# 0xPolygonZero/proof-protocol-decoder

Measured on AMD Instinct MI355X. Metric: txn-proofs/sec (whole node), 256-txn synthetic block, higher is better.
Workload: dtype u64 (Goldilocks field)

## Files before the change

include/bpg.h:

```cpp
#ifndef BPG_H
#define BPG_H
#include <stddef.h>
#include <stdint.h>

#ifdef __cplusplus
extern "C" {
#endif

typedef enum {
  BP_OK = 0,
  BP_ERR_ABORTED = -1,
  BP_ERR_INVALID_INPUT = -2,
  BP_ERR_RANGE = -3,
  BP_ERR_DEVICE = -4,
  BP_ERR_VERIFY = -5,
  BP_ERR_UNSUPPORTED = -6
} bp_status;

const char* bp_last_error(void);
const char* bp_version(void);
int bp_device_count(void);
int bp_use_blocking_sync(int device);
int bp_host_wait_mode(int device);



#define BP_NTT_MAX_COLS 65535u

enum { BP_NTT_FWD_BR2NAT = 0, BP_NTT_INV_NAT2BR = 1, BP_NTT_FWD_NAT = 2, BP_NTT_INV_NAT = 3 };
int bp_ntt_batch(uint64_t* d_cols, uint32_t log_n, uint32_t n_cols, uint64_t col_stride, int dir,
                 void* stream);

int bp_intt_batch(const uint64_t* d_values, uint64_t in_stride, uint64_t* d_coeffs_out, uint64_t out_stride,
                  uint32_t log_n, uint32_t n_cols, void* stream);

int bp_lde_batch(const uint64_t* d_in, uint64_t in_stride, uint64_t* d_coeffs_out, uint64_t coeffs_stride,
                 uint64_t* d_lde_out, uint64_t lde_stride, uint32_t log_n, uint32_t rate_bits,
                 uint32_t n_cols, int from_coeffs, void* stream);

int bp_debug_copy_u64(const uint64_t* d_in, uint64_t* d_out, uint64_t n, void* stream);

int bp_debug_field_ops(const uint64_t* d_a, const uint64_t* d_b, uint64_t* d_out, uint64_t n, void* stream);
int bp_debug_mul_pow2(const uint64_t* d_a, uint64_t* d_out, uint64_t n, void* stream);

void bp_tune_quad_threshold(uint64_t n_perms);
void bp_tune_merkle_fused(int mode);
void bp_tune_merkle_wide(int log2_parents);
void bp_tune_poseidon_mx(int on);
void bp_tune_poseidon_mx_sets(int sets);
void bp_tune_poseidon_grouped(int on);
void bp_tune_assume_loaded(int mode);
void bp_tune_rec_batch(int n);
void bp_tune_side_lanes(int n);
void bp_tune_rec_riders(int on);
void bp_tune_witness_threads(int n);
void bp_tune_host_wait(int mode);
void bp_tune_host_poseidon(int mode);
int bp_debug_poseidon_host(uint64_t* states, size_t n);
void bp_tune_k5_spread(int on);
uint32_t bp_debug_poseidon_group_ops(uint32_t K);
int bp_debug_poseidon_group_tables(uint32_t K, uint32_t r0, uint8_t* out_ops, int32_t* out_cform, int32_t* out_cmain,
                                   int32_t* out_max_plane_sum);

void bp_tune_ntt_split(int mode);
void bp_tune_ntt_mx(int mode);
void bp_tune_reset(void);
int bp_debug_tune_state(char* buf, size_t cap);
int bp_debug_ntt_mx_tables(int kind, int inverse, uint8_t* out_a, int32_t* out_c, uint64_t* out_tw256,
                           uint64_t* out_tw16);
int bp_debug_poseidon_mx_cin(uint32_t* out);

int bp_poseidon_perm_batch(uint64_t* d_states, uint64_t n, void* stream);

uint64_t bp_merkle_digest_words(uint32_t log_leaves, uint32_t cap_height);
int bp_merkle_commit(const uint64_t* d_lde, uint64_t lde_stride, uint32_t n_cols, uint32_t log_n,
                     uint32_t rate_bits, uint32_t cap_height, uint64_t* d_digests, void* stream);

struct bp_stark_cfg;
typedef struct bp_air_family {
  uint32_t first_index, count;
  uint32_t kind;
  uint32_t degree;
} bp_air_family;
typedef struct bp_air_desc {
  uint32_t air_id;
  char name[24];
  uint32_t fixed_n_cols;
  uint32_t n_const_max;
  uint32_t degree;
  uint32_t n_cols, n_aux;
  uint32_t n_air_constraints, n_ctl_constraints;
  uint32_t n_units;
  uint32_t n_families;
  bp_air_family families[24];
} bp_air_desc;
uint32_t bp_air_count(void);
int bp_air_describe(uint32_t air_id, uint32_t n_cols, uint32_t n_const, uint32_t deg_pow, bp_air_desc* out);

int bp_air_register(const uint64_t* program, size_t n_words, uint32_t* air_id_out);
int bp_air_unregister(uint32_t air_id);
int bp_air_program_digest(uint32_t air_id, uint8_t out[32]);

uint64_t bp_quotient_scratch_words(uint32_t air_id, const struct bp_stark_cfg* shape);
int bp_quotient_eval(uint32_t air_id, const struct bp_stark_cfg* shape, const uint64_t* d_trace_lde,
                     const uint64_t* d_aux_lde, const uint64_t* d_const_lde, const uint64_t ctl[4],
                     const uint64_t alphas[2], uint64_t* d_scratch, uint64_t* d_qvals_out, void* stream);

int bp_air_port_products(uint32_t air_id, const struct bp_stark_cfg* shape, const uint64_t* d_trace, uint64_t stride,
                         const uint64_t* d_consts, const uint64_t pub[4], const uint64_t ctl[4], uint64_t* d_aux_out, void* stream);

int bp_debug_air_aux(uint32_t air_id, const struct bp_stark_cfg* shape, const uint64_t* d_trace, const uint64_t ctl[4],
                     uint64_t* d_aux_out, void* stream);

typedef struct bp_air_violation {
  uint32_t row, constraint, family, kind;
  uint64_t value;
} bp_air_violation;
int bp_air_check_trace(uint32_t air_id, const struct bp_stark_cfg* shape, const uint64_t* d_trace, uint64_t stride,
                       const uint64_t* d_consts, const uint64_t pub[4], uint32_t max_rows, uint64_t* n_violated_rows,
                       uint32_t* rows_out, bp_air_violation* viol_out, uint32_t max_viol, uint32_t* n_viol, void* stream);
int bp_air_check_trace_host(uint32_t air_id, const struct bp_stark_cfg* shape, const uint64_t* trace, uint64_t stride,
                            const uint64_t* consts, const uint64_t pub[4], uint32_t max_rows, uint64_t* n_violated_rows,
                            uint32_t* rows_out, bp_air_violation* viol_out, uint32_t max_viol, uint32_t* n_viol);

int bp_keccak_trace(const uint64_t* d_inputs, uint64_t seed, uint32_t log_n, uint64_t* d_trace_out, void* stream);
int bp_logic_trace(const uint64_t* d_inputs, uint64_t seed, uint32_t log_n, uint64_t* d_trace_out, void* stream);
int bp_memory_trace(const uint64_t* d_inputs, uint64_t seed, uint32_t log_n, uint64_t* d_trace_out, void* stream);
int bp_arithmetic_trace(const uint64_t* d_inputs, uint64_t seed, uint32_t log_n, uint64_t* d_trace_out, void* stream);
int bp_byte_packing_trace(const uint64_t* d_inputs, uint64_t seed, uint32_t log_n, uint64_t* d_trace_out, void* stream);
int bp_keccak_sponge_trace(const uint64_t* d_inputs, uint64_t seed, uint32_t log_n, uint64_t* d_trace_out, void* stream);
int bp_arithmetic_mul_trace(const uint64_t* d_inputs, uint64_t seed, uint32_t log_n, uint64_t* d_trace_out, void* stream);

typedef struct bp_plonk_layout {
  uint32_t pi_len, n_paths, path_depth, path_pi0;
  uint32_t leaf_len;
} bp_plonk_layout;
int bp_plonk_constants(uint64_t seed, uint32_t log_n, const bp_plonk_layout* layout, uint64_t* d_consts_out, void* stream);
int bp_plonk_trace(const uint64_t* d_consts, uint64_t seed, const uint64_t* pi, const bp_plonk_layout* layout, const uint64_t* paths,
                   uint32_t log_n, uint64_t* d_trace_out, void* stream);

int bp_fri_fold(const uint64_t* d_values, uint32_t log_nl, uint32_t rate_bits, uint32_t arity_bits, uint64_t shift,
                const uint64_t beta[2], uint64_t* d_out, void* stream);

int bp_openings(const uint64_t* d_coeffs, uint64_t stride, uint32_t log_n, uint32_t n_cols, const uint64_t z0[2],
                const uint64_t z1[2], uint64_t* d_pw_scratch, uint64_t* d_out, void* stream);

int bp_pow_grind(const uint64_t state[12], uint32_t pos, uint32_t bits, uint64_t* nonce_out, void* stream);

typedef struct bp_stark_cfg {
  uint32_t log_n, n_cols, n_const, deg_pow, rate_bits, cap_height, num_queries, pow_bits, arity_bits,
      final_poly_bits;
} bp_stark_cfg;
int bp_stark_prove_synthetic(const bp_stark_cfg* cfg, uint64_t seed, uint64_t const_seed, int device,
                             uint8_t** out, size_t* out_len);
int bp_stark_prove_air(uint32_t air_id, const bp_stark_cfg* cfg, uint64_t seed, uint64_t const_seed, int device,
                       uint8_t** out, size_t* out_len);
int bp_stark_prove_trace(uint32_t air_id, const bp_stark_cfg* cfg, const uint64_t* d_trace, uint64_t stride,
                         const uint64_t* d_consts, const uint64_t* pub, int device, uint8_t** out, size_t* out_len);
int bp_stark_verify_air(uint32_t air_id, const bp_stark_cfg* cfg, const uint64_t* const_cap, const uint8_t* proof,
                        size_t len);
void bp_stark_public_inputs(uint64_t seed, uint64_t out[4]);
void bp_stark_public_input_list(uint64_t seed, uint64_t out[4]);
int bp_stark_verify_air_pub(uint32_t air_id, const bp_stark_cfg* cfg, const uint64_t* const_cap, const uint64_t* pub,
                            const uint8_t* proof, size_t len);
typedef struct bp_set_table {
  uint32_t air_id;
  bp_stark_cfg cfg;
  const uint64_t* d_trace;
  uint64_t stride;
  const uint64_t* d_consts;
  const uint64_t* pub;
} bp_set_table;
typedef struct bp_set_port {
  uint32_t table, port;
} bp_set_port;
typedef struct bp_set_link {
  uint32_t n_looking;
  bp_set_port looking[8];
  bp_set_port looked;
} bp_set_link;
#define BP_SET_SKIP_LINK_CHECK 1u
int bp_stark_prove_table_set(const bp_set_table* tables, uint32_t n_tables, const bp_set_link* links, uint32_t n_links,
                             uint32_t flags, int device, uint8_t** out, size_t* out_len);
int bp_stark_verify_table_set(const bp_set_table* statement, uint32_t n_tables, const uint64_t* const* const_caps,
                              const bp_set_link* links, uint32_t n_links, const uint8_t* proof, size_t len);
void bp_release_cached_memory(void);
void bp_free_buffer(uint8_t* buf);

#define BP_NUM_TABLES 7

typedef struct bp_config {
  uint32_t table_log_lo[BP_NUM_TABLES], table_log_hi[BP_NUM_TABLES];
  uint32_t stark_rate_bits, stark_cap_height, stark_num_queries, stark_pow_bits, arity_bits, final_poly_bits;
  uint32_t rec_log_n, rec_n_cols, rec_n_const, rec_rate_bits, rec_num_queries, rec_pow_bits;
  uint32_t shrink_depth;
  uint32_t rec_air_id;
  int32_t device;
  uint32_t n_workers;
  uint64_t arena_bytes;
} bp_config;
// ... 161 lines not shown
```

proof_protocol_decoder_amd/_lib.py:

```python
import ctypes as C
import os

_HERE = os.path.dirname(os.path.abspath(__file__))
_PATH = os.environ.get("BPG_LIBBPG") or os.path.join(_HERE, "lib", "libbpg.so")

BP_OK = 0
STATUS_NAMES = {0: "BP_OK", -1: "BP_ERR_ABORTED", -2: "BP_ERR_INVALID_INPUT", -3: "BP_ERR_RANGE",
                -4: "BP_ERR_DEVICE", -5: "BP_ERR_VERIFY", -6: "BP_ERR_UNSUPPORTED"}


class BpgError(RuntimeError):

    def __init__(self, code, message):
        super().__init__("%s: %s" % (STATUS_NAMES.get(code, str(code)), message))
        self.code = code
        self.message = message


class StarkCfg(C.Structure):
    _fields_ = [(n, C.c_uint32) for n in ("log_n", "n_cols", "n_const", "deg_pow", "rate_bits", "cap_height",
                                           "num_queries", "pow_bits", "arity_bits", "final_poly_bits")]


class AirFamily(C.Structure):
    _fields_ = [(n, C.c_uint32) for n in ("first_index", "count", "kind", "degree")]


class AirDesc(C.Structure):
    _fields_ = ([("air_id", C.c_uint32), ("name", C.c_char * 24)]
                + [(n, C.c_uint32) for n in ("fixed_n_cols", "n_const_max", "degree", "n_cols", "n_aux",
                                             "n_air_constraints", "n_ctl_constraints", "n_units", "n_families")]
                + [("families", AirFamily * 24)])


class SetTable(C.Structure):
    _fields_ = [("air_id", C.c_uint32), ("cfg", StarkCfg), ("d_trace", C.c_void_p), ("stride", C.c_uint64),
                ("d_consts", C.c_void_p), ("pub", C.POINTER(C.c_uint64))]


class SetPort(C.Structure):
    _fields_ = [("table", C.c_uint32), ("port", C.c_uint32)]


class SetLink(C.Structure):
    _fields_ = [("n_looking", C.c_uint32), ("looking", SetPort * 8), ("looked", SetPort)]


BP_SET_SKIP_LINK_CHECK = 1


class AirViolation(C.Structure):
    _fields_ = [(n, C.c_uint32) for n in ("row", "constraint", "family", "kind")] + [("value", C.c_uint64)]


def take_buffer(ptr, length):
    try:
        return C.string_at(ptr, length.value)
    finally:
        lib().bp_free_buffer(ptr)


def lib_path():
    return _PATH


KNOBS = ("quad_threshold", "assume_loaded", "merkle_fused", "merkle_wide", "poseidon_mx", "poseidon_mx_sets",
         "poseidon_grouped", "ntt_mx", "ntt_split", "k5_spread", "host_wait", "host_poseidon", "rec_batch",
         "witness_threads", "side_lanes")

_lib = None


def lib():
    global _lib
    if _lib is not None:
        return _lib
    if not os.path.exists(_PATH):
        raise ImportError(
            "libbpg.so not built at %s -- run `python -c 'import __graft_entry__ as g; g.build()'` "
            "(hipcc --offload-arch=gfx950). There is no CPU fallback for the hot path." % _PATH)
    L = C.CDLL(_PATH)
    vp, u32, u64, i = C.c_void_p, C.c_uint32, C.c_uint64, C.c_int
    L.bp_last_error.restype = C.c_char_p
    L.bp_version.restype = C.c_char_p
    L.bp_device_count.restype = i
    L.bp_ntt_batch.argtypes = [vp, u32, u32, u64, i, vp]
    L.bp_intt_batch.argtypes = [vp, u64, vp, u64, u32, u32, vp]
    L.bp_lde_batch.argtypes = [vp, u64, vp, u64, vp, u64, u32, u32, u32, i, vp]
    L.bp_poseidon_perm_batch.argtypes = [vp, u64, vp]
    L.bp_debug_field_ops.argtypes = [vp, vp, vp, u64, vp]
    L.bp_debug_mul_pow2.argtypes = [vp, vp, u64, vp]
    L.bp_quotient_scratch_words.argtypes = [u32, C.POINTER(StarkCfg)]
    L.bp_quotient_scratch_words.restype = u64
    L.bp_quotient_eval.argtypes = [u32, C.POINTER(StarkCfg), vp, vp, vp, C.POINTER(u64), C.POINTER(u64), vp, vp, vp]
    L.bp_air_count.restype = u32
    L.bp_air_describe.argtypes = [u32, u32, u32, u32, C.POINTER(AirDesc)]
    check_args = [u32, C.POINTER(StarkCfg), vp, u64, vp, C.POINTER(u64), u32, C.POINTER(u64), C.POINTER(u32),
                  C.POINTER(AirViolation), u32, C.POINTER(u32)]
    L.bp_air_check_trace.argtypes = check_args + [vp]
    L.bp_air_check_trace_host.argtypes = check_args
    L.bp_keccak_trace.argtypes = [vp, u64, u32, vp, vp]
    L.bp_logic_trace.argtypes = [vp, u64, u32, vp, vp]
    L.bp_memory_trace.argtypes = [vp, u64, u32, vp, vp]
    L.bp_arithmetic_trace.argtypes = [vp, u64, u32, vp, vp]
    L.bp_byte_packing_trace.argtypes = [vp, u64, u32, vp, vp]
    L.bp_keccak_sponge_trace.argtypes = [vp, u64, u32, vp, vp]
    L.bp_arithmetic_mul_trace.argtypes = [vp, u64, u32, vp, vp]
    L.bp_stark_verify_air.argtypes = [u32, C.POINTER(StarkCfg), C.POINTER(u64), C.c_char_p, C.c_size_t]
    L.bp_stark_prove_air.argtypes = [u32, C.POINTER(StarkCfg), u64, u64, i, C.POINTER(C.POINTER(C.c_uint8)),
                                     C.POINTER(C.c_size_t)]
    L.bp_stark_verify_air_pub.argtypes = [u32, C.POINTER(StarkCfg), C.POINTER(u64), C.POINTER(u64), C.c_char_p, C.c_size_t]
    L.bp_stark_prove_trace.argtypes = [u32, C.POINTER(StarkCfg), vp, u64, vp, C.POINTER(u64), i, C.POINTER(C.POINTER(C.c_uint8)),
                                       C.POINTER(C.c_size_t)]
    L.bp_debug_air_aux.argtypes = [u32, C.POINTER(StarkCfg), vp, C.POINTER(u64), vp, vp]
    L.bp_air_port_products.argtypes = [u32, C.POINTER(StarkCfg), vp, u64, vp, C.POINTER(u64), C.POINTER(u64), vp, vp]
    L.bp_stark_prove_table_set.argtypes = [C.POINTER(SetTable), u32, C.POINTER(SetLink), u32, u32, i,
                                           C.POINTER(C.POINTER(C.c_uint8)), C.POINTER(C.c_size_t)]
    L.bp_stark_verify_table_set.argtypes = [C.POINTER(SetTable), u32, C.POINTER(C.POINTER(u64)), C.POINTER(SetLink), u32,
                                            C.c_char_p, C.c_size_t]
    L.bp_air_register.argtypes = [vp, C.c_size_t, C.POINTER(u32)]
    L.bp_air_unregister.argtypes = [u32]
    L.bp_air_program_digest.argtypes = [u32, C.c_char_p]
    L.bp_fri_fold.argtypes = [vp, u32, u32, u32, u64, C.POINTER(u64), vp, vp]
    L.bp_openings.argtypes = [vp, u64, u32, u32, C.POINTER(u64), C.POINTER(u64), vp, vp, vp]
    L.bp_pow_grind.argtypes = [C.POINTER(u64), u32, u32, C.POINTER(u64), vp]
    L.bp_merkle_digest_words.argtypes = [u32, u32]
    L.bp_merkle_digest_words.restype = u64
    L.bp_merkle_commit.argtypes = [vp, u64, u32, u32, u32, u32, vp, vp]
    L.bp_stark_prove_synthetic.argtypes = [C.POINTER(StarkCfg), u64, u64, i, C.POINTER(C.POINTER(C.c_uint8)),
                                           C.POINTER(C.c_size_t)]
    L.bp_free_buffer.argtypes = [C.POINTER(C.c_uint8)]
    L.bp_free_buffer.restype = None
    for knob in KNOBS:
        fn = getattr(L, "bp_tune_" + knob)
        fn.argtypes = [u64 if knob == "quad_threshold" else i]
        fn.restype = None
    L.bp_tune_reset.argtypes = []
    L.bp_tune_reset.restype = None
    L.bp_debug_tune_state.argtypes = [C.c_char_p, C.c_size_t]
    _lib = L
    return L


def check(rc):
    if rc != BP_OK:
        raise BpgError(rc, lib().bp_last_error().decode("utf-8", "replace"))
```

proof_protocol_decoder_amd/csrc/hash_kernels.hip:

```cpp
#include <atomic>
#include <cstring>
#include <memory>
#include <mutex>
#include <vector>
#include "common.hpp"
#include "poseidon.cuh"
#include "poseidon_mx.cuh"
#include "stark_kernels.hpp"
#include "tune.hpp"

namespace {

__global__ void __launch_bounds__(256) perm_batch_kernel(uint64_t* __restrict__ states, uint64_t n) {
  uint64_t i = blockIdx.x * (uint64_t)blockDim.x + threadIdx.x;
  if (i >= n) return;
  uint64_t s[12];
#pragma unroll
  for (int k = 0; k < 12; k++) s[k] = states[i * 12 + k];
  poseidon::permute(s);
#pragma unroll
  for (int k = 0; k < 12; k++) states[i * 12 + k] = gl::canon(s[k]);
}

__global__ void __launch_bounds__(256) __attribute__((amdgpu_waves_per_eu(4, 8)))
// ... 258 lines not shown
      const uint64_t leaf = ((uint64_t)gl::bitrev(t, rate_bits) << log_n) | gl::bitrev(mm, log_n);
      digests[leaf * 4 + kb] = gl::canon(e[m][0]);
    }
  }
}

template <int NS, bool GR>
__global__ void BPG_MX_BOUNDS
merkle_level_mx_kernel(const uint64_t* __restrict__ child, uint64_t* __restrict__ parent, uint64_t n_parents,
                       uint64_t* __restrict__ mirror, uint64_t dig_bstride, const uint32_t* __restrict__ gtab) {
  if (gridDim.x * gridDim.z <= 64) __builtin_amdgcn_s_setprio(3);
  child += blockIdx.z * dig_bstride;
  parent += blockIdx.z * dig_bstride;
  if (mirror) mirror += blockIdx.z * n_parents * 4;
  BPG_MX_TABLES(NS, GR, gtab)
  const poseidon::mx::Ctx c = poseidon::mx::make_ctx(cin);
  const uint64_t base = ((uint64_t)blockIdx.x * 4 + (threadIdx.x >> 6)) * (16 * NS) + (threadIdx.x & 15);
  uint64_t e[NS][3];
#pragma unroll
  for (int m = 0; m < NS; m++) {
    const uint64_t i = base + 16 * m < n_parents ? base + 16 * m : n_parents - 1;
    e[m][0] = child[i * 8 + c.kb];
    e[m][1] = child[i * 8 + 4 + c.kb];
    e[m][2] = 0;
  }
  BPG_MX_PERMUTE(NS, GR, e, c, gtab)
#pragma unroll
  for (int m = 0; m < NS; m++) {
    const uint64_t i = base + 16 * m;
    if (i < n_parents) {
      const uint64_t d = gl::canon(e[m][0]);
      parent[i * 4 + c.kb] = d;
      if (mirror) mirror[i * 4 + c.kb] = d;
    }
  }
}

__global__ void __launch_bounds__(256)
merkle_subtree_mx_kernel(const uint64_t* __restrict__ child, uint64_t* __restrict__ out, uint64_t n_parents,
                         uint32_t levels, uint64_t* __restrict__ mirror, uint64_t dig_bstride) {
  if (gridDim.x * gridDim.z <= 64) __builtin_amdgcn_s_setprio(3);
  child += blockIdx.z * dig_bstride;
  out += blockIdx.z * dig_bstride;
  if (mirror) mirror += blockIdx.z * ((n_parents >> (levels - 1)) * 4);
  __shared__ __attribute__((aligned(16))) uint32_t cin[poseidon::mx::CIN_WORDS];
  __shared__ uint64_t sm[2][64 * 4];
  poseidon::mx::build_cin(cin);
  __syncthreads();
  const poseidon::mx::Ctx c = poseidon::mx::make_ctx(cin);
  const uint32_t wave = threadIdx.x >> 6, n = threadIdx.x & 15;
  uint64_t level_parents = n_parents;
  uint32_t wg_parents = n_parents < 64 ? (uint32_t)n_parents : 64u;
  uint64_t wg_first = (uint64_t)blockIdx.x * 64;
  uint64_t* dst = out;
  for (uint32_t l = 0; l < levels; l++) {
    if (wave * 16 < wg_parents) {
      const uint32_t q = wave * 16 + n, qc = q < wg_parents ? q : wg_parents - 1;
      uint64_t e[1][3];
      if (l == 0) {
        e[0][0] = child[(wg_first + qc) * 8 + c.kb];
        e[0][1] = child[(wg_first + qc) * 8 + 4 + c.kb];
      } else {
        e[0][0] = sm[(l - 1) & 1][(2 * qc) * 4 + c.kb];
        e[0][1] = sm[(l - 1) & 1][(2 * qc + 1) * 4 + c.kb];
      }
      e[0][2] = 0;
      poseidon::mx::permute<1>(e, c);
      if (q < wg_parents) {
        const uint64_t d = gl::canon(e[0][0]);
        dst[(wg_first + q) * 4 + c.kb] = d;
        if (mirror && l + 1 == levels) mirror[(wg_first + q) * 4 + c.kb] = d;
        sm[l & 1][q * 4 + c.kb] = d;
      }
    }
    __syncthreads();
    dst += level_parents * 4;
    level_parents >>= 1;
    wg_parents >>= 1;
    wg_first >>= 1;
  }
}

__global__ void __launch_bounds__(256)
merkle_subtree_wide_kernel(const uint64_t* __restrict__ child, uint64_t* __restrict__ out, uint64_t n_parents,
                           uint32_t levels, uint64_t* __restrict__ mirror, uint64_t dig_bstride) {
  if (gridDim.x * gridDim.z <= 64) __builtin_amdgcn_s_setprio(3);
  child += blockIdx.z * dig_bstride;
  out += blockIdx.z * dig_bstride;
  if (mirror) mirror += blockIdx.z * ((n_parents >> (levels - 1)) * 4);
  __shared__ __attribute__((aligned(16))) uint32_t cin[poseidon::mx::CIN_WORDS];
  __shared__ uint64_t sm[2][256 * 4];
  poseidon::mx::build_cin(cin);
  __syncthreads();
  const poseidon::mx::Ctx c = poseidon::mx::make_ctx(cin);
  const uint32_t wave = threadIdx.x >> 6, n = threadIdx.x & 15;
  uint64_t level_parents = n_parents;
  uint32_t wg_parents = n_parents < 256 ? (uint32_t)n_parents : 256u;
  uint64_t wg_first = (uint64_t)blockIdx.x * 256;
  uint64_t* dst = out;
  for (uint32_t l = 0; l < levels; l++) {
    const uint64_t* prev = sm[(l - 1) & 1];
    if (wg_parents >= 64) {
      if (wave * 64 < wg_parents) {
        uint64_t e[4][3];
#pragma unroll
        for (int m = 0; m < 4; m++) {
          const uint32_t q = wave * 64 + 16 * m + n;
          if (l == 0) {
            e[m][0] = child[(wg_first + q) * 8 + c.kb];
            e[m][1] = child[(wg_first + q) * 8 + 4 + c.kb];
          } else {
            e[m][0] = prev[(2 * q) * 4 + c.kb];
            e[m][1] = prev[(2 * q + 1) * 4 + c.kb];
          }
          e[m][2] = 0;
        }
        poseidon::mx::permute<4>(e, c);
#pragma unroll
        for (int m = 0; m < 4; m++) {
          const uint32_t q = wave * 64 + 16 * m + n;
          const uint64_t d = gl::canon(e[m][0]);
          dst[(wg_first + q) * 4 + c.kb] = d;
          if (mirror && l + 1 == levels) mirror[(wg_first + q) * 4 + c.kb] = d;
          sm[l & 1][q * 4 + c.kb] = d;
        }
      }
    } else if (wave * 16 < wg_parents) {
      const uint32_t q = wave * 16 + n, qc = q < wg_parents ? q : wg_parents - 1;
      uint64_t e[1][3];
      if (l == 0) {
        e[0][0] = child[(wg_first + qc) * 8 + c.kb];
        e[0][1] = child[(wg_first + qc) * 8 + 4 + c.kb];
      } else {
        e[0][0] = prev[(2 * qc) * 4 + c.kb];
        e[0][1] = prev[(2 * qc + 1) * 4 + c.kb];
      }
      e[0][2] = 0;
      poseidon::mx::permute<1>(e, c);
      if (q < wg_parents) {
        const uint64_t d = gl::canon(e[0][0]);
        dst[(wg_first + q) * 4 + c.kb] = d;
        if (mirror && l + 1 == levels) mirror[(wg_first + q) * 4 + c.kb] = d;
        sm[l & 1][q * 4 + c.kb] = d;
      }
    }
    __syncthreads();
    dst += level_parents * 4;
    level_parents >>= 1;
    wg_parents >>= 1;
    wg_first >>= 1;
  }
}

template <int K>
__device__ __forceinline__ void mul_pow2_planes(const uint64_t (&x)[4], uint64_t* __restrict__ out, uint64_t n, uint64_t i0) {
  uint64_t r4[4], r3[3];
  const uint64_t x3[3] = {x[1], x[2], x[3]};
  gl::mul_pow2_n<12 * K, 4>(x, r4);
  __builtin_amdgcn_sched_barrier(0);
  gl::mul_pow2_n<12 * K, 3>(x3, r3);
  __builtin_amdgcn_sched_barrier(0);
#pragma unroll
  for (int k = 0; k < 4; k++) {
    const uint64_t i = i0 + k;
    if (i >= n) break;
    out[(3 * (K - 1) + 0) * n + i] = gl::canon(r4[k]);
    out[(3 * (K - 1) + 1) * n + i] = k ? gl::canon(r3[k - 1]) : gl::canon(r4[0]);
    out[(3 * (K - 1) + 2) * n + i] = gl::canon(gl::mul_pow2(x[k], 12 * K));
  }
  if constexpr (K < 7) mul_pow2_planes<K + 1>(x, out, n, i0);
}
__global__ void __launch_bounds__(256) mul_pow2_kernel(const uint64_t* __restrict__ a, uint64_t* __restrict__ out, uint64_t n) {
  const uint64_t i0 = (blockIdx.x * (uint64_t)blockDim.x + threadIdx.x) * 4;
  if (i0 >= n) return;
  uint64_t x[4];
#pragma unroll
  for (int k = 0; k < 4; k++) x[k] = a[i0 + k < n ? i0 + k : n - 1];
  mul_pow2_planes<1>(x, out, n, i0);
}

__global__ void __launch_bounds__(256)
calib_copy_u64_kernel(const uint64_t* __restrict__ in, uint64_t* __restrict__ out, uint64_t n) {
  uint64_t i = blockIdx.x * (uint64_t)blockDim.x + threadIdx.x;
  const uint64_t stride = (uint64_t)gridDim.x * blockDim.x;
  for (; i < n; i += stride) out[i] = in[i];
}

__global__ void __launch_bounds__(256) field_ops_kernel(const uint64_t* __restrict__ a, const uint64_t* __restrict__ b,
                                                        uint64_t* __restrict__ out, uint64_t n) {
  const uint64_t i0 = (blockIdx.x * (uint64_t)blockDim.x + threadIdx.x) * 4;
  if (i0 >= n) return;
  uint64_t x[4], y[4];
#pragma unroll
  for (int k = 0; k < 4; k++) {
    const uint64_t i = i0 + k < n ? i0 + k : n - 1;
    x[k] = a[i];
    y[k] = b[i];
  }
  uint64_t r4[4], r3[3];
  gl::mul_n<4>(x, y, r4);
  __builtin_amdgcn_sched_barrier(0);
  const uint64_t x3[3] = {x[1], x[2], x[3]}, y3[3] = {y[1], y[2], y[3]};
  gl::mul_n<3>(x3, y3, r3);
  __builtin_amdgcn_sched_barrier(0);
  gl::DotAcc d[4] = {gl::dot_zero(), gl::dot_zero(), gl::dot_zero(), gl::dot_zero()};
  gl::dot_mad4(d, x, y);
  __builtin_amdgcn_sched_barrier(0);
  gl::dot_mad4(d, y, x);
  __builtin_amdgcn_sched_barrier(0);
  const uint64_t yy[4] = {y[0], y[0], y[0], y[0]};
  gl::dot_mad4(d, x, yy);
  __builtin_amdgcn_sched_barrier(0);
  uint64_t cy[4] = {y[0], y[1], y[2], y[3]}, sum4[4], dif4[4], cx4[4] = {x[0], x[1], x[2], x[3]};
  gl::canon_n<4>(cy);
  __builtin_amdgcn_sched_barrier(0);
  gl::add_n<4>(x, cy, sum4);
  __builtin_amdgcn_sched_barrier(0);
  gl::sub_n<4>(x, cy, dif4);
  __builtin_amdgcn_sched_barrier(0);
  gl::canon_n<4>(cx4);
  __builtin_amdgcn_sched_barrier(0);
#pragma unroll
  for (int k = 0; k < 4; k++) {
    const uint64_t i = i0 + k;
    if (i >= n) break;
    const uint64_t cb = gl::canon(y[k]);
    out[0 * n + i] = gl::canon(gl::mul(x[k], y[k]));
    out[1 * n + i] = gl::canon(r4[k]);
    out[2 * n + i] = k ? gl::canon(r3[k - 1]) : gl::canon(r4[0]);
    uint64_t lo, hi;
    gl::mul_wide(x[k], y[k], lo, hi);
    out[3 * n + i] = gl::canon(gl::reduce128(lo, hi));
    out[4 * n + i] = gl::canon(gl::add(x[k], cb));
    out[5 * n + i] = gl::canon(gl::sub(x[k], cb));
    out[6 * n + i] = gl::dot_reduce(d[k]);
    out[7 * n + i] = gl::canon(gl::mul7(x[k]));
    out[8 * n + i] = gl::inv(gl::canon(x[k]));
    const gl::Ext e = gl::mul(gl::Ext{gl::canon(x[k]), cb}, gl::Ext{cb, gl::canon(x[k] ^ y[k])});
    out[9 * n + i] = e.c0;
    out[10 * n + i] = e.c1;
    out[11 * n + i] = gl::canon(sum4[k]);
    out[12 * n + i] = gl::canon(dif4[k]);
    out[13 * n + i] = cx4[k];
    out[14 * n + i] = cy[k];
  }
}

}

namespace bpg {

static std::atomic<int> g_active_provers{0};
void prover_active(int delta) { g_active_provers.fetch_add(delta, std::memory_order_relaxed); }
int provers_active() { return g_active_provers.load(std::memory_order_relaxed); }
bool device_loaded() {
  const int a = tune().assume_loaded.load(std::memory_order_relaxed);
  return a < 0 ? g_active_provers.load(std::memory_order_relaxed) >= 6 : a != 0;
}
bool poseidon_mx() { return tune().poseidon_mx.load(std::memory_order_relaxed) != 0; }
uint64_t quad_threshold() {
  const uint64_t t = tune().quad_threshold.load(std::memory_order_relaxed);
  if (t) return t;
  const bool loaded = device_loaded();
  if (poseidon_mx()) return (uint64_t)1 << (loaded ? 13 : 19);
  return (uint64_t)1 << (loaded ? 13 : 17);
}
int mx_sets(uint64_t n) {
  if (!poseidon_mx()) return 0;
  const int f = tune().poseidon_mx_sets.load(std::memory_order_relaxed);
  if (f) return f;
  const uint64_t t = quad_threshold();
  return n >= t ? 4 : (n >= t / 2 ? 2 : 1);
}
static std::mutex g_group_mu;
static const uint32_t* g_group_dev[16] = {};
static std::atomic<int> g_group_state[16];
static std::vector<uint32_t>* g_group_image = nullptr;

static bool build_group_image() {
  namespace pg = poseidon::group;
  namespace gx = poseidon::mx::grp;
  if (g_group_image) return true;
  auto img = std::make_unique<std::vector<uint32_t>>(gx::IMAGE_WORDS, 0);
  for (int g = 0; g < gx::N_GROUPS; g++) {
    pg::Tables t;
    uint32_t* c = img->data() + gx::OPS_WORDS + g * gx::C_WORDS;
    if (g < 2) {
      if (!pg::build(gx::K, 4 + gx::K * g, &t) || (int)t.ops.size() != gx::LAY.n_ops * 1024) return false;
      if (g == 0) std::memcpy(img->data(), t.ops.data(), t.ops.size());
      else if (std::memcmp(img->data(), t.ops.data(), t.ops.size()) != 0) return false;
    } else {
      constexpr pg::Layout L6 = pg::layout(gx::SHORT_K);
      if (!pg::build(gx::SHORT_K, 20, &t) || (int)t.ops.size() != L6.n_ops * 1024) return false;
      const uint8_t* o8 = reinterpret_cast<const uint8_t*>(img->data());
      for (int i = 0; i < L6.main_base; i++) {
        const int j = i < L6.d_base[1] ? i : gx::LAY.d_base[1] + (i - L6.d_base[1]);
        for (int b = 0; b < 1024; b++) {
          const uint8_t v6 = t.ops[(size_t)i * 1024 + b], v8 = o8[(size_t)j * 1024 + b];
          const int row = (b >> 4) & 15;
          const bool blank = i >= L6.w_base[1] && row >= 8;
          if (blank ? v6 != 0 : v6 != v8) return false;
        }
      }
      std::memcpy(img->data() + gx::TABLE_WORDS, t.ops.data() + (size_t)L6.main_base * 1024, 18 * 1024);
    }
    std::memcpy(c, t.cform.data(), pg::CFORM_WORDS * 4);
    std::memcpy(c + pg::CFORM_WORDS, t.cmain.data(), pg::CMAIN_WORDS * 4);
  }
  static const uint32_t MC[12] = {17, 15, 41, 16, 2, 28, 13, 13, 39, 18, 34, 20};
  uint32_t* am = img->data() + gx::OPS_WORDS + gx::N_GROUPS * gx::C_WORDS;
  for (uint32_t g = 0; g < 3; g++)
    for (uint32_t lane = 0; lane < 64; lane++)
      for (uint32_t a = 0; a < 3; a++) {
        const uint32_t r = lane & 15, kb = lane >> 4, i = (r >> 2) + 4 * g, k = kb + 4 * a;
        am[(g * 64 + lane) * 4 + a] = (MC[(k + 12 - i) % 12] + ((i | k) == 0 ? 8u : 0u)) << (8 * (r & 3));
      }
  g_group_image = img.release();
  return true;
}
const uint32_t* group_tables() {
  if (!tune().poseidon_grouped.load(std::memory_order_relaxed)) return nullptr;
  int dev = 0;
  if (hipGetDevice(&dev) != hipSuccess || dev < 0 || dev >= 16) return nullptr;
  std::atomic<int>& state = g_group_state[dev];
  const uint32_t*& slot = g_group_dev[dev];
  if (state.load(std::memory_order_acquire) > 0) return slot;
  std::lock_guard<std::mutex> lk(g_group_mu);
  if (const int st = state.load(std::memory_order_acquire)) return st > 0 ? slot : nullptr;
  void* d = nullptr;
  const size_t bytes = (size_t)poseidon::mx::grp::IMAGE_WORDS * 4;
  if (!build_group_image() || hipMalloc(&d, bytes) != hipSuccess ||
      hipMemcpy(d, g_group_image->data(), bytes, hipMemcpyHostToDevice) != hipSuccess) {
    if (d) (void)hipFree(d);
    state.store(-1, std::memory_order_release);
    return nullptr;
  }
  slot = static_cast<const uint32_t*>(d);
  state.store(1, std::memory_order_release);
  return slot;
}

#define BPG_MX_DISPATCH(NS_EXPR, KERNEL, ITEMS, BATCH, ...)                                                 \
  switch (NS_EXPR) {                                                                                       \
    case 4:                                                                                                \
      if (const uint32_t* gtab_ = bpg::group_tables())                                                     \
        KERNEL<4, true><<<dim3(ceil_div((ITEMS), 256), 1, (BATCH)), 256, 0, st>>>(__VA_ARGS__, gtab_);    \
      else                                                                                                 \
        KERNEL<4, false><<<dim3(ceil_div((ITEMS), 256), 1, (BATCH)), 256, 0, st>>>(__VA_ARGS__, nullptr); \
      break;                                                                                               \
    case 2: KERNEL<2, false><<<dim3(ceil_div((ITEMS), 128), 1, (BATCH)), 256, 0, st>>>(__VA_ARGS__, nullptr); break; \
    default: KERNEL<1, false><<<dim3(ceil_div((ITEMS), 64), 1, (BATCH)), 256, 0, st>>>(__VA_ARGS__, nullptr); break; \
  }

int merkle_upper_levels(uint64_t* d_digests, uint32_t log_leaves, uint32_t cap_height, hipStream_t st,
                        uint64_t* mirror, bool* mirrored, uint32_t batch, uint64_t dig_bstride) {
  uint64_t* lvl = d_digests;
  uint32_t l = log_leaves;
  if (mirrored) *mirrored = false;
  if (batch == 0 || batch > MAX_BATCH) return fail(BP_ERR_INVALID_INPUT, "merkle: batch of %u trees", batch);
  while (l > cap_height) {
    const uint64_t cnt = (uint64_t)1 << l, parents = cnt / 2;
    uint64_t* nxt = lvl + cnt * 4;
    const int fmode = tune().merkle_fused.load(std::memory_order_relaxed);
    constexpr uint64_t flimit = 2048;
    const bool fused = parents <= flimit && parents < quad_threshold() && (fmode > 0 || (fmode < 0 && !device_loaded()));
    const uint64_t wlimit = (uint64_t)1 << tune().merkle_wide.load(std::memory_order_relaxed);
    if (!fused && fmode > 0 && poseidon_mx() && parents >= 256 && parents <= wlimit && parents % 256 == 0) {
      uint32_t levels = l - cap_height;
      if (levels > 9) levels = 9;
      uint64_t* mir = (l - levels == cap_height) ? mirror : nullptr;
      merkle_subtree_wide_kernel<<<dim3((uint32_t)(parents / 256), 1, batch), 256, 0, st>>>(lvl, nxt, parents, levels, mir, dig_bstride);
      BPG_LAUNCH_CHECK();
      if (mir && mirrored) *mirrored = true;
      for (uint32_t k = 0; k < levels; k++) {
        lvl += ((uint64_t)1 << l) * 4;
        l--;
      }
      continue;
    }
    if (!fused) {
      uint64_t* mir = (l - 1 == cap_height) ? mirror : nullptr;
      if (const int ns = mx_sets(parents * batch)) {
        BPG_MX_DISPATCH(ns, merkle_level_mx_kernel, parents, batch, lvl, nxt, parents, mir, dig_bstride)
      } else if (parents * batch >= quad_threshold())
        merkle_level_kernel<<<dim3(ceil_div(parents, 256), 1, batch), 256, 0, st>>>(lvl, nxt, parents, mir, dig_bstride);
      else
        merkle_level_quad_kernel<<<dim3(ceil_div(cnt * 2, 256), 1, batch), 256, 0, st>>>(lvl, nxt, parents, mir, dig_bstride);
      BPG_LAUNCH_CHECK();
      if (mir && mirrored) *mirrored = true;
      lvl = nxt;
      l--;
      continue;
    }
    uint32_t levels = l - cap_height;
    const uint32_t wgs = parents >= 64 ? (uint32_t)(parents / 64) : 1;
    uint32_t max_levels = 1;
    for (uint64_t p = parents >= 64 ? 64 : parents; p > 1; p >>= 1) max_levels++;
    if (levels > max_levels) levels = max_levels;
    uint64_t* mir = (l - levels == cap_height) ? mirror : nullptr;
    if (poseidon_mx()) merkle_subtree_mx_kernel<<<dim3(wgs, 1, batch), 256, 0, st>>>(lvl, nxt, parents, levels, mir, dig_bstride);
    else merkle_subtree_quad_kernel<<<dim3(wgs, 1, batch), 256, 0, st>>>(lvl, nxt, parents, levels, mir, dig_bstride);
    BPG_LAUNCH_CHECK();
    if (mir && mirrored) *mirrored = true;
    for (uint32_t k = 0; k < levels; k++) {
      lvl += ((uint64_t)1 << l) * 4;
      l--;
    }
  }
  return BP_OK;
}

int merkle_commit_rows(const uint64_t* d_leaves, uint32_t leaf_len, uint32_t log_leaves, uint32_t cap_height,
                       uint64_t* d_digests, hipStream_t st) {
  uint64_t n = (uint64_t)1 << log_leaves;
  leaf_hash_rows_kernel<<<ceil_div(n, 256), 256, 0, st>>>(d_leaves, leaf_len, n, d_digests);
  BPG_LAUNCH_CHECK();
  return merkle_upper_levels(d_digests, log_leaves, cap_height, st, nullptr, nullptr);
}

}

extern "C" {

int bp_debug_copy_u64(const uint64_t* d_in, uint64_t* d_out, uint64_t n, void* stream) {
  if (!d_in || !d_out) return bpg::fail(BP_ERR_INVALID_INPUT, "bp_debug_copy_u64: null buffer");
  calib_copy_u64_kernel<<<4096, 256, 0, bpg::as_stream(stream)>>>(d_in, d_out, n);
  BPG_LAUNCH_CHECK();
  return BP_OK;
}

int bp_debug_field_ops(const uint64_t* d_a, const uint64_t* d_b, uint64_t* d_out, uint64_t n, void* stream) {
  if (!n) return BP_OK;
  if (!d_a || !d_b || !d_out) return bpg::fail(BP_ERR_INVALID_INPUT, "bp_debug_field_ops: null buffer");
  field_ops_kernel<<<bpg::ceil_div(bpg::ceil_div(n, 4), 256), 256, 0, bpg::as_stream(stream)>>>(d_a, d_b, d_out, n);
  BPG_LAUNCH_CHECK();
  return BP_OK;
}

int bp_debug_mul_pow2(const uint64_t* d_a, uint64_t* d_out, uint64_t n, void* stream) {
  if (!n) return BP_OK;
  if (!d_a || !d_out) return bpg::fail(BP_ERR_INVALID_INPUT, "bp_debug_mul_pow2: null buffer");
  mul_pow2_kernel<<<bpg::ceil_div(bpg::ceil_div(n, 4), 256), 256, 0, bpg::as_stream(stream)>>>(d_a, d_out, n);
  BPG_LAUNCH_CHECK();
  return BP_OK;
}

int bp_debug_poseidon_mx_cin(uint32_t* out) {
  if (!out) return bpg::fail(BP_ERR_INVALID_INPUT, "bp_debug_poseidon_mx_cin: null buffer");
  static const poseidon::mx::CinTable t = poseidon::mx::make_cin_table();
  for (int i = 0; i < poseidon::mx::CIN_WORDS; i++) out[i] = t.v[i];
  return BP_OK;
}

uint32_t bp_debug_poseidon_group_ops(uint32_t K) { return K >= 2 && K <= 8 ? (uint32_t)poseidon::group::layout((int)K).n_ops : 0; }
int bp_debug_poseidon_group_tables(uint32_t K, uint32_t r0, uint8_t* out_ops, int32_t* out_cform, int32_t* out_cmain,
                                   int32_t* out_max_plane_sum) try {
  if (!out_ops || !out_cform || !out_cmain) return bpg::fail(BP_ERR_INVALID_INPUT, "bp_debug_poseidon_group_tables: null output");
  poseidon::group::Tables t;
  if (!poseidon::group::build((int)K, (int)r0, &t))
    return bpg::fail(BP_ERR_INVALID_INPUT, "bp_debug_poseidon_group_tables: no such group (K=%u r0=%u)", K, r0);
  std::memcpy(out_ops, t.ops.data(), t.ops.size());
  std::memcpy(out_cform, t.cform.data(), t.cform.size() * 4);
  std::memcpy(out_cmain, t.cmain.data(), t.cmain.size() * 4);
  if (out_max_plane_sum) *out_max_plane_sum = t.max_plane_sum;
  return BP_OK;
}
BPG_ABI_CATCH("bp_debug_poseidon_group_tables")

uint64_t bp_merkle_digest_words(uint32_t log_leaves, uint32_t cap_height) {
  return (((uint64_t)2 << log_leaves) - ((uint64_t)1 << cap_height)) * 4;
}

int bp_poseidon_perm_batch(uint64_t* d_states, uint64_t n, void* stream) try {
  if (!n) return BP_OK;
  if (!d_states) return bpg::fail(BP_ERR_INVALID_INPUT, "bp_poseidon_perm_batch: null buffer");
  hipStream_t st = bpg::as_stream(stream);
  using bpg::ceil_div;
  if (const int ns = bpg::mx_sets(n)) {
    BPG_MX_DISPATCH(ns, perm_batch_mx_kernel, n, 1, d_states, n)
  } else
    perm_batch_kernel<<<bpg::ceil_div(n, 256), 256, 0, st>>>(d_states, n);
  BPG_LAUNCH_CHECK();
  return BP_OK;
}
BPG_ABI_CATCH("bp_poseidon_perm_batch")

int bp_merkle_commit(const uint64_t* d_lde, uint64_t lde_stride, uint32_t n_cols, uint32_t log_n,
                     uint32_t rate_bits, uint32_t cap_height, uint64_t* d_digests, void* stream) try {
  return bpg::merkle_commit_cols(d_lde, lde_stride, n_cols, log_n, rate_bits, cap_height, d_digests,
                                 bpg::as_stream(stream), nullptr, nullptr, 1, 0, 0);
}
BPG_ABI_CATCH("bp_merkle_commit")

}

namespace bpg {

int merkle_commit_cols(const uint64_t* d_lde, uint64_t lde_stride, uint32_t n_cols, uint32_t log_n, uint32_t rate_bits,
                       uint32_t cap_height, uint64_t* d_digests, hipStream_t st, uint64_t* mirror, bool* mirrored,
                       uint32_t batch, uint64_t lde_bstride, uint64_t dig_bstride) {
  const uint32_t log_leaves = log_n + rate_bits;
  if (!d_lde || !d_digests) return fail(BP_ERR_INVALID_INPUT, "bp_merkle_commit: null buffer");
  if (log_leaves > 30 || cap_height > log_leaves || n_cols == 0 || lde_stride < ((uint64_t)1 << log_leaves))
    return fail(BP_ERR_INVALID_INPUT,
                "bp_merkle_commit: bad shape (log_n=%u rate_bits=%u cap_height=%u n_cols=%u stride=%llu)", log_n,
                rate_bits, cap_height, n_cols, (unsigned long long)lde_stride);
  if (batch == 0 || batch > MAX_BATCH) return fail(BP_ERR_INVALID_INPUT, "merkle: batch of %u trees", batch);
  uint64_t rows = (uint64_t)1 << log_leaves;
  {
    KernelTimer kt(PROF_LEAF_HASH, st, n_cols > 4 ? (double)batch * (double)rows * (double)((n_cols + 7) / 8) : 0.0);
    int ns = mx_sets(rows * batch);
    while (ns > 1 && (uint64_t)16 * ns > rows) ns >>= 1;
    if (ns && rows >= 16) {
      BPG_MX_DISPATCH(ns, leaf_hash_mx_kernel, rows, batch, d_lde, lde_stride, n_cols, log_n, rate_bits, d_digests, lde_bstride, dig_bstride)
    } else if (rows * batch < quad_threshold())
      leaf_hash_quad_kernel<<<dim3(ceil_div(rows * 4, 256), 1, batch), 256, 0, st>>>(d_lde, lde_stride, n_cols, log_n, rate_bits,
                                                                               d_digests, lde_bstride, dig_bstride);
    else
      leaf_hash_kernel<<<dim3(ceil_div(rows, 256), 1, batch), 256, 0, st>>>(d_lde, lde_stride, n_cols, log_n, rate_bits, d_digests,
                                                                      lde_bstride, dig_bstride);
  }
  BPG_LAUNCH_CHECK();
  return merkle_upper_levels(d_digests, log_leaves, cap_height, st, mirror, mirrored, batch, dig_bstride);
}

}
```

proof_protocol_decoder_amd/csrc/poseidon_mx.cuh:

```cuda
#pragma once
#include "poseidon.cuh"
#include "poseidon_group.hpp"

namespace poseidon {
namespace mx {

using mxa::v4i;

constexpr int CIN_PER_ROUND = 4 * 24;
constexpr int CIN_WORDS = 30 * CIN_PER_ROUND;

__device__ __forceinline__ uint32_t mds_entry(uint32_t i, uint32_t k) {
  constexpr uint32_t C[12] = {17, 15, 41, 16, 2, 28, 13, 13, 39, 18, 34, 20};
  const uint32_t d = (k + 12 - i) % 12;
  uint32_t v = 0;
#pragma unroll
  for (int j = 0; j < 12; j++) v = d == (uint32_t)j ? C[j] : v;
  return v + ((i | k) == 0 ? 8u : 0u);
}

struct CinTable {
  uint32_t v[CIN_WORDS];
};
constexpr CinTable make_cin_table() {
// ... 178 lines not shown
__device__ __forceinline__ v4i at_global(const v4i* image, uint32_t off) {
  return *(__attribute__((address_space(1))) const v4i*)((__attribute__((address_space(1))) const char*)image + off);
}

template <int ROW, int SLOT>
__device__ __forceinline__ void put_sigma(v4i& b, uint64_t y) {
  b[SLOT] = __builtin_amdgcn_update_dpp(b[SLOT], (int)(uint32_t)y, 0xE4, 1 << ROW, 0xF, false);
  b[SLOT + 1] = __builtin_amdgcn_update_dpp(b[SLOT + 1], (int)(uint32_t)(y >> 32), 0xE4, 1 << ROW, 0xF, false);
}

struct State {
  v4i blo[4], bhi[4], bsig[4];
  v4i acc[4][2];
};
__device__ __forceinline__ void init_state(State& s) {
#pragma unroll
  for (int m = 0; m < 4; m++) {
    s.blo[m] = v4i{0, 0, 0, 0};
    s.bhi[m] = v4i{0, 0, 0, 0};
    s.bsig[m] = v4i{0, 0, 0, 0};
  }
}

template <int J>
__device__ __forceinline__ void step(State& s, uint64_t (&e)[4][3], const v4i* ops, const int* cform, const Lanes& o,
                                     uint32_t kb, bool full = true) {
  constexpr int P = J / 4, F = J % 4;
  if constexpr (F == 0) {
    constexpr int nw = LAY.w_per_half[P];
#pragma unroll
    for (int half = 0; half < 2; half++) {
      const v4i* cf = (const v4i*)(cform + (P * 2 + half) * 16);
      const v4i* w = ops + (LAY.w_base[P] + half * nw) * 64;
#pragma unroll
      for (int m = 0; m < 4; m++) {
        s.acc[m][half] = __builtin_amdgcn_mfma_i32_16x16x64_i8(at(w, o.w[m]), s.blo[m], cf[(kb - m) & 3], 0, 0, 0);
        s.acc[m][half] = __builtin_amdgcn_mfma_i32_16x16x64_i8(at(w + 64, o.w[m]), s.bhi[m], s.acc[m][half], 0, 0, 0);
        if constexpr (P > 0)
          s.acc[m][half] = __builtin_amdgcn_mfma_i32_16x16x64_i8(at(w + 128, o.d[m]), s.bsig[m], s.acc[m][half], 0, 0, 0);
      }
    }
  }
  uint32_t l[4], h[4];
  if constexpr (J == 0) {
#pragma unroll
    for (int m = 0; m < 4; m++) { l[m] = (uint32_t)e[m][0]; h[m] = (uint32_t)(e[m][0] >> 32); }
    gather0(l, h);
  } else {
    v4i dl = s.acc[(4 - F) & 3][0], dh = s.acc[(4 - F) & 3][1];
#pragma unroll
    for (int g = 1; g < 4; g++) {
      const bool here = kb == (uint32_t)g;
#pragma unroll
      for (int q = 0; q < 4; q++) {
        dl[q] = here ? s.acc[(g - F + 4) & 3][0][q] : dl[q];
        dh[q] = here ? s.acc[(g - F + 4) & 3][1][q] : dh[q];
      }
    }
    const uint64_t x = mxa::reduce_row(planes(dl), planes(dh));
    l[0] = (uint32_t)x;
    h[0] = (uint32_t)(x >> 32);
  }
  const uint64_t y = sbox(gl::cc::mk64(l[0], h[0])) ^ 0x8080808080808080ULL;
  put_sigma<(F + 0) & 3, 2 * P>(s.bsig[0], y);
  put_sigma<(F + 1) & 3, 2 * P>(s.bsig[1], y);
  put_sigma<(F + 2) & 3, 2 * P>(s.bsig[2], y);
  put_sigma<(F + 3) & 3, 2 * P>(s.bsig[3], y);
  if constexpr (J >= LAY.d_first[P] && J < LAY.d_first[P] + LAY.d_count[P]) {
    if (J == SHORT_K - 1 && !full) return;
#pragma unroll
    for (int half = 0; half < 2; half++) {
      const v4i* a = ops + (LAY.d_base[P] + 2 * (J - LAY.d_first[P]) + half) * 64;
#pragma unroll
      for (int m = 0; m < 4; m++)
        s.acc[m][half] = __builtin_amdgcn_mfma_i32_16x16x64_i8(at(a, o.d[m]), s.bsig[m], s.acc[m][half], 0, 0, 0);
    }
  }
}

__device__ __forceinline__ void partial_group(State& s, Lanes& o, uint64_t (&e)[4][3], const uint32_t* tab,
                                              const uint32_t* __restrict__ gtab, int grp) {
  const uint32_t lane = threadIdx.x & 63, kb = lane >> 4;
  const bool full = grp < 2;
  const v4i* ops = (const v4i*)tab;
  const int* cform = (const int*)(tab + OPS_WORDS + grp * C_WORDS);
  const int* cmain = cform + poseidon::group::CFORM_WORDS;
  renew(o);
#pragma unroll
  for (int m = 0; m < 4; m++) {
#pragma unroll
    for (int a = 0; a < 3; a++) {
      s.blo[m][a] = (int)((uint32_t)e[m][a] ^ 0x80808080u);
      s.bhi[m][a] = (int)((uint32_t)(e[m][a] >> 32) ^ 0x80808080u);
    }
  }
  step<0>(s, e, ops, cform, o, kb);
  step<1>(s, e, ops, cform, o, kb);
  step<2>(s, e, ops, cform, o, kb);
  step<3>(s, e, ops, cform, o, kb);
  step<4>(s, e, ops, cform, o, kb);
  step<5>(s, e, ops, cform, o, kb, full);
  if (full) {
    step<6>(s, e, ops, cform, o, kb);
    step<7>(s, e, ops, cform, o, kb);
  }
  const v4i* lops = ops + LAY.main_base * 64;
  const v4i* gops = (const v4i*)(gtab + TABLE_WORDS);
#pragma unroll
  for (int g = 0; g < 3; g++) {
    v4i d[4][2];
#pragma unroll
    for (int h = 0; h < 2; h++) {
      const int t = (g * 2 + h) * 3 * 64;
      v4i a_lo, a_hi, a_sg[4];
      if (full) {
        a_lo = at(lops + t, o.s[0]);
        a_hi = at(lops + t + 64, o.s[0]);
#pragma unroll
        for (int m = 0; m < 4; m++) a_sg[m] = at(lops + t + 128, o.s[m]);
      } else {
        a_lo = at_global(gops + t, o.s[0]);
        a_hi = at_global(gops + t + 64, o.s[0]);
#pragma unroll
        for (int m = 0; m < 4; m++) a_sg[m] = at_global(gops + t + 128, o.s[m]);
      }
      const v4i c0 = ((const v4i*)(cmain + (g * 2 + h) * 16))[kb];
#pragma unroll
      for (int m = 0; m < 4; m++) {
        d[m][h] = __builtin_amdgcn_mfma_i32_16x16x64_i8(a_lo, s.blo[m], c0, 0, 0, 0);
        d[m][h] = __builtin_amdgcn_mfma_i32_16x16x64_i8(a_hi, s.bhi[m], d[m][h], 0, 0, 0);
        d[m][h] = __builtin_amdgcn_mfma_i32_16x16x64_i8(a_sg[m], s.bsig[m], d[m][h], 0, 0, 0);
      }
    }
    uint64_t L[4], H[4], x[4];
#pragma unroll
    for (int m = 0; m < 4; m++) { L[m] = planes(d[m][0]); H[m] = planes(d[m][1]); }
    reduce_rows<4>(L, H, x);
#pragma unroll
    for (int m = 0; m < 4; m++) e[m][g] = x[m];
  }
}
}

constexpr int CIN_GROUPED_ROUNDS = 8;
constexpr int CIN_GROUPED_WORDS = CIN_GROUPED_ROUNDS * CIN_PER_ROUND;
__device__ __forceinline__ int cin_slot(int rnd) { return rnd < 4 ? rnd : rnd - (30 - CIN_GROUPED_ROUNDS); }
__device__ __forceinline__ void build_cin_grouped(uint32_t* __restrict__ cin) {
  const uint4* src = (const uint4*)CIN_TABLE.v;
  uint4* dst = (uint4*)cin;
  for (uint32_t i = threadIdx.x; i < (uint32_t)CIN_GROUPED_WORDS / 4; i += blockDim.x)
    dst[i] = src[i < 4 * CIN_PER_ROUND / 4 ? i : i + (30 - CIN_GROUPED_ROUNDS) * CIN_PER_ROUND / 4];
}

__device__ __forceinline__ void mds4_lds(uint64_t (&e)[4][3], const Ctx& c, int rnd, const uint32_t* tab) {
  const v4i* cr = (const v4i*)(c.cin + cin_slot(rnd) * CIN_PER_ROUND);
  const v4i* am = (const v4i*)(tab + grp::OPS_WORDS + grp::N_GROUPS * grp::C_WORDS) + (threadIdx.x & 63);
#pragma unroll
  for (int m = 0; m < 4; m++) {
    v4i blo, bhi;
#pragma unroll
    for (int a = 0; a < 3; a++) {
      blo[a] = (int)((uint32_t)e[m][a] ^ 0x80808080u);
      bhi[a] = (int)((uint32_t)(e[m][a] >> 32) ^ 0x80808080u);
    }
    blo[3] = 0;
    bhi[3] = 0;
    uint64_t L[3], H[3];
#pragma unroll
    for (int g = 0; g < 3; g++) {
      const v4i A = am[g * 64];
      const v4i dl = __builtin_amdgcn_mfma_i32_16x16x64_i8(A, blo, cr[2 * g], 0, 0, 0);
      const v4i dh = __builtin_amdgcn_mfma_i32_16x16x64_i8(A, bhi, cr[2 * g + 1], 0, 0, 0);
      L[g] = planes(dl);
      H[g] = planes(dh);
    }
    reduce_rows<3>(L, H, e[m]);
  }
}

__device__ __forceinline__ void permute_grouped(uint64_t (&e)[4][3], const Ctx& c, const uint32_t* tab,
                                                const uint32_t* __restrict__ gtab) {
#pragma unroll
  for (int a = 0; a < 3; a++) {
    const uint64_t k = RC[c.kb + 4 * a];
#pragma unroll
    for (int m = 0; m < 4; m++) e[m][a] = gl::add(e[m][a], k);
  }
  int rnd = 0;
#pragma unroll 1
  for (int k = 0; k < 4; k++, rnd++) {
    sbox_full<4>(e);
    mds4_lds(e, c, rnd, tab);
  }
  grp::State s;
  grp::init_state(s);
  grp::Lanes o = grp::lanes_of(threadIdx.x & 63);
#pragma unroll 1
  for (int g = 0; g < grp::N_GROUPS; g++) grp::partial_group(s, o, e, tab, gtab, g);
  rnd = 26;
#pragma unroll 1
  for (int k = 0; k < 4; k++, rnd++) {
    sbox_full<4>(e);
    mds4_lds(e, c, rnd, tab);
  }
}

template <int NS>
__device__ __forceinline__ void permute(uint64_t (&e)[NS][3], const Ctx& c) {
#pragma unroll
  for (int a = 0; a < 3; a++) {
    const uint64_t k = RC[c.kb + 4 * a];
#pragma unroll
    for (int m = 0; m < NS; m++) e[m][a] = gl::add(e[m][a], k);
  }
  int rnd = 0;
#pragma unroll 1
  for (int k = 0; k < 4; k++, rnd++) {
    sbox_full<NS>(e);
    mds<NS>(e, c, rnd);
  }
#pragma unroll 1
  for (int k = 0; k < 22; k++, rnd++) {
    sbox_word0<NS>(e, c);
    mds<NS>(e, c, rnd);
  }
#pragma unroll 1
  for (int k = 0; k < 4; k++, rnd++) {
    sbox_full<NS>(e);
    mds<NS>(e, c, rnd);
  }
}

}
}
```

proof_protocol_decoder_amd/csrc/proofgen.cpp:

```cpp
#include <algorithm>
#include <atomic>
#include <condition_variable>
#include <cstdlib>
#include <memory>
#include <mutex>
#include <string>
#include <system_error>
#include <thread>
#include <deque>
#include <random>
#include <set>
#include <unordered_map>
#include "air_check.hpp"
#include "mpt.hpp"
#include "prover.hpp"
#include "rec_pool.hpp"
#include "tune.hpp"
#include "txn_tables.hpp"

using namespace bpg;
using namespace bpg::txn;
extern "C" int bp_use_blocking_sync(int device);
extern "C" int bp_host_wait_mode(int device);

// ... 310 lines not shown
  if (rc.air_id == air::PLONK) std::memcpy(ctl.pub, pi_hash, sizeof(pi_hash));
  return stark_verify(rc, circ.cap.data(), ctl, ch, b.stark, b.stark_words);
}

constexpr size_t SEEN_MAX = 8192;
void remember_proof(const bp_state* s, const uint8_t* bytes, size_t len) {
  const mpt::H256 h = mpt::keccak256(bytes, len);
  std::lock_guard<std::mutex> lk(s->seen_mu);
  if (!s->seen.insert(h).second) return;
  s->seen_order.push_back(h);
  if (s->seen_order.size() > SEEN_MAX) {
    s->seen.erase(s->seen_order.front());
    s->seen_order.pop_front();
  }
}
bool produced_here(const bp_state* s, const uint8_t* bytes, size_t len) {
  const mpt::H256 h = mpt::keccak256(bytes, len);
  std::lock_guard<std::mutex> lk(s->seen_mu);
  return s->seen.count(h) != 0;
}

int verify_foreign(const bp_state* s, const Box& b, const char* what) {
  if (b.circuit != CIRCUIT_ROOT + b.kind)
    return fail(BP_ERR_VERIFY, "%s was made by circuit %llu, expected %u", what, (unsigned long long)b.circuit,
                CIRCUIT_ROOT + (uint32_t)b.kind);
  for (size_t i = 0; i < b.n_pi; i++)
    if (b.pi[i] >= gl::P) return fail(BP_ERR_VERIFY, "%s: non-canonical public input", what);
  LightCircuit lc;
  lc.cap = s->special[b.kind].consts.cap;
  std::memcpy(lc.digest, s->special[b.kind].digest, 32);
  int r = rec_verify(s->rec_cfg, lc, b);
  if (r) {
    const std::string why = bp_last_error();
    return fail(BP_ERR_VERIFY, "%s does not verify: %s", what, why.c_str());
  }
  return BP_OK;
}

int verify_child(const bp_state* s, const Box& b, const char* what, const uint8_t* bytes, size_t len) {
  return produced_here(s, bytes, len) ? BP_OK : verify_foreign(s, b, what);
}

int box_of_job(const bp_state* s, const RecJob& job, const std::vector<uint64_t>& words, TreeBuf* out) {
  if (int r = emit_box(job.kind, CIRCUIT_ROOT + job.kind, job.pi, words, &out->p, &out->n)) return r;
  remember_proof(s, out->p, out->n);
  return BP_OK;
}
int finish_job(const bp_state* s, const RecJob& job, const std::vector<uint64_t>& words, RecPool* pool) {
  TreeBuf b;
  if (int r = box_of_job(s, job, words, &b)) return r;
  pool->complete(job, b.p, b.n);
  return BP_OK;
}

}

extern "C" {

void bp_config_default(bp_config* c) {
  static const uint32_t lo[BP_NUM_TABLES] = {16, 9, 12, 14, 9, 12, 17}, hi[BP_NUM_TABLES] = {28, 28, 28, 25, 25, 28, 30};
  std::memset(c, 0, sizeof(*c));
  for (int t = 0; t < BP_NUM_TABLES; t++) { c->table_log_lo[t] = lo[t]; c->table_log_hi[t] = hi[t]; }
  c->stark_rate_bits = 1; c->stark_cap_height = 4; c->stark_num_queries = 84; c->stark_pow_bits = 16;
  c->arity_bits = 4; c->final_poly_bits = 5;
  c->rec_log_n = 13; c->rec_n_cols = 135; c->rec_n_const = 85; c->rec_rate_bits = 3; c->rec_num_queries = 28;
  c->rec_pow_bits = 16;
  c->shrink_depth = 3;
  c->rec_air_id = 8;
  c->device = 0; c->n_workers = 4; c->arena_bytes = (uint64_t)6 << 30;
}

int bp_state_build(const bp_config* cfg, bp_state** out) try {
  if (!cfg || !out) return fail(BP_ERR_INVALID_INPUT, "bp_state_build: null argument");
  *out = nullptr;
  const StarkCfg rc = rec_cfg_of(*cfg);
  int r = check_cfg(rc);
  if (r) return r;
  if (cfg->shrink_depth < 1)
    return fail(BP_ERR_INVALID_INPUT, "shrink_depth must be at least 1: the root circuit walks Merkle paths of the recursion shape's depth, "
                "so its children are recursion-shaped proofs, not the tables' STARK proofs");
  uint32_t n_circ = 0;
  for (int t = 0; t < BP_NUM_TABLES; t++) {
    if (cfg->table_log_lo[t] >= cfg->table_log_hi[t] || cfg->table_log_hi[t] > 31)
      return fail(BP_ERR_INVALID_INPUT, "empty or invalid range for table %s", TABLES[t].name);
    StarkCfg tc = table_cfg_of(*cfg, cfg->table_log_lo[t], 8);
    if ((r = check_cfg(tc))) return r;
    n_circ += cfg->table_log_hi[t] - cfg->table_log_lo[t];
  }
  if (cfg->n_workers == 0 || cfg->n_workers > 64) return fail(BP_ERR_INVALID_INPUT, "n_workers out of range");
  int n_dev = bp_device_count();
  if (n_dev <= 0) return fail(BP_ERR_DEVICE, "no HIP device visible: the hot path has no CPU fallback");
  if (cfg->device < 0 || cfg->device >= n_dev) return fail(BP_ERR_DEVICE, "device %d not present", cfg->device);
  (void)bp_use_blocking_sync(cfg->device);
  std::unique_ptr<bp_state> s(new bp_state());
  s->cfg = *cfg;
  s->rec_cfg = rc;
  const uint64_t N = (uint64_t)1 << rc.log_n, M = N << rc.rate_bits;
  const size_t per = ((size_t)rc.n_const * (2 * N + M) + 2 * M * 4 + 4096) * 8;
  const size_t circuits_bytes = per * (n_circ + 3 + BP_NUM_TABLES) + (64u << 20);
  {
    (void)hipSetDevice(cfg->device);
    size_t free_b = 0, total_b = 0;
    BPG_HIP(hipMemGetInfo(&free_b, &total_b));
    const double need = (double)circuits_bytes + (double)cfg->n_workers * (double)cfg->arena_bytes;
    if (need > (double)free_b)
      return fail(BP_ERR_DEVICE,
                  "prover state does not fit device %d: %u preprocessed circuits %.1f GiB + %u prover arenas x %.1f GiB = "
                  "%.1f GiB, %.1f GiB free of %.1f GiB (lower n_workers or arena_bytes, or narrow the table ranges)",
                  cfg->device, n_circ + 3 + BP_NUM_TABLES, circuits_bytes / 1073741824.0, cfg->n_workers,
                  cfg->arena_bytes / 1073741824.0, need / 1073741824.0, free_b / 1073741824.0, total_b / 1073741824.0);
  }
  struct Unbuild {
    std::unique_ptr<bp_state>& s;
    ~Unbuild() {
      if (!s) return;
      for (auto& w : s->workers) w->destroy();
      s->builder.destroy();
    }
  } unbuild{s};
  if ((r = s->builder.init(cfg->device, circuits_bytes))) return r;
  s->table_circuits.resize(n_circ);
  uint32_t idx = 0;
  for (int t = 0; t < BP_NUM_TABLES; t++) {
    s->table_offset[t] = idx;
    for (uint32_t d = cfg->table_log_lo[t]; d < cfg->table_log_hi[t]; d++, idx++)
      if ((r = build_circuit(s->builder, rc, circuit_seed(t, d),
                             air::plonk::Layout{CHAIN_PATH_PI0 + 8, 1, d + cfg->stark_rate_bits - cfg->stark_cap_height, CHAIN_PATH_PI0},
                             &s->table_circuits[idx]))) return r;
  }
  const uint32_t depth = rc.log_n + rc.rate_bits - rc.cap_height;
  auto with_leaf = [&](air::plonk::Layout lay) {
    air::plonk::Layout l = lay;
    l.leaf_len = rc.n_cols;
    return (rc.air_id == air::PLONK && air::plonk::layout_ok(l, 1u << rc.log_n)) ? l : lay;
  };
  for (int t = 0; t < BP_NUM_TABLES; t++)
    if ((r = build_circuit(s->builder, rc, circuit_seed(t, SHRINK_SEED_DEGREE), with_leaf(air::plonk::Layout{CHAIN_PATH_PI0 + 8, 1, depth, CHAIN_PATH_PI0}),
                           &s->shrink_circuits[t]))) return r;
  air::plonk::Layout special[3] = {with_leaf({ROOT_PATH_PI0 + 8 * BP_NUM_TABLES + BP_PV_WORDS, BP_NUM_TABLES, depth, ROOT_PATH_PI0}),
                                   with_leaf({AGG_PATH_PI0 + 2 * 8 + BP_PV_WORDS, 2, depth, AGG_PATH_PI0}),
                                   with_leaf({BLOCK_PATH_PI0 + 8 + BP_PV_WORDS, 1, depth, BLOCK_PATH_PI0})};
  for (uint32_t k = 0; k < 3; k++)
    if ((r = build_circuit(s->builder, rc, circuit_seed(CIRCUIT_ROOT + k, 0), special[k], &s->special[k]))) return r;
  BPG_HIP(hipStreamSynchronize(s->builder.stream));
  for (uint32_t i = 0; i < cfg->n_workers; i++) {
    std::unique_ptr<Worker> w(new Worker());
    if ((r = w->init(cfg->device, cfg->arena_bytes))) { w->destroy(); return r; }
    s->idle.push_back(w.get());
    s->workers.push_back(std::move(w));
  }
  {
    const char* env = std::getenv("GPU_MAX_HW_QUEUES");
    const long queues = env && *env ? std::strtol(env, nullptr, 10) : 4;
    if (queues < (long)cfg->n_workers) {
      char buf[512];
      std::snprintf(buf, sizeof(buf),
                    "GPU_MAX_HW_QUEUES is %s%ld but this state has %u prover streams: HIP maps a process's streams onto that many "
                    "hardware queues, so concurrent bp_generate_* calls beyond it serialise (measured: 16 streams on 4 queues run at "
                    "about half the rate).  Set GPU_MAX_HW_QUEUES >= n_workers (bench.py uses 32) in the environment BEFORE the process "
                    "makes its first HIP call.",
                    env && *env ? "" : "unset = ", queues, cfg->n_workers);
      s->warnings = buf;
    }
    if (bp_host_wait_mode(cfg->device) == 2) {
      if (!s->warnings.empty()) s->warnings += "\n";
      s->warnings += "The process had used this device before the library's first call, so the device's host-wait mode was left alone "
                     "(bp_use_blocking_sync); the library's prover threads wait with their own poll-and-sleep loop instead of the "
                     "runtime's spinning wait.  Nothing to do; call bp_use_blocking_sync(device) first thing for interrupt-driven waits.";
    }
  }
  *out = s.release();
  return BP_OK;
}
BPG_ABI_CATCH("bp_state_build")

const char* bp_state_warnings(const bp_state* s) { return s ? s->warnings.c_str() : ""; }
int bp_state_config(const bp_state* s, bp_config* out) {
  if (!s || !out) return fail(BP_ERR_INVALID_INPUT, "bp_state_config: null argument");
  *out = s->cfg;
  return BP_OK;
}

void bp_state_free(bp_state* s) {
  if (!s) return;
  (void)hipSetDevice(s->cfg.device);
  for (auto& w : s->workers) w->destroy();
  s->builder.destroy();
  delete s;
}

uint64_t bp_state_device_bytes(const bp_state* s) {
  if (!s) return 0;
  return s->builder.arena.capacity() + (uint64_t)s->workers.size() * s->cfg.arena_bytes;
}

int bp_state_root_after(const uint64_t root_before[4], uint64_t seed, uint64_t txn_number, uint64_t out[4]) {
  if (!root_before || !out) return fail(BP_ERR_INVALID_INPUT, "bp_state_root_after: null argument");
  for (int i = 0; i < 4; i++) if (root_before[i] >= gl::P) return fail(BP_ERR_INVALID_INPUT, "non-canonical state root");
  root_after(root_before, seed, txn_number, out);
  return BP_OK;
}

int bp_proof_public_values(const uint8_t* proof, size_t len, uint64_t pv_out[BP_PV_WORDS], int* kind_out) try {
  if (!proof || len % 8 || len < (BOX_HDR + BP_PV_WORDS) * 8) return fail(BP_ERR_INVALID_INPUT, "proof: truncated");
  const uint64_t* w = reinterpret_cast<const uint64_t*>(proof);
  if (w[0] != PROOF_BOX_MAGIC || w[1] > 2 || w[2] < BP_PV_WORDS || w[2] > air::plonk::MAX_PI || len / 8 < BOX_HDR + w[2])
    return fail(BP_ERR_INVALID_INPUT, "proof: bad header");
  if (pv_out) std::memcpy(pv_out, w + BOX_HDR + w[2] - BP_PV_WORDS, BP_PV_WORDS * 8);
  if (kind_out) *kind_out = (int)w[1];
  return BP_OK;
}
BPG_ABI_CATCH("bp_proof_public_values")

struct TableProofs {
  StarkCfg tcfg[BP_NUM_TABLES];
  std::vector<uint64_t> pv;
  Ctl ctl;
  std::vector<uint64_t> proof[BP_NUM_TABLES];
  uint64_t first_leaf[BP_NUM_TABLES][4];
};
static int build_traces(Worker& w, const uint64_t* I, const TxnWitness* wit, const StarkCfg tcfg[BP_NUM_TABLES],
                        uint64_t* d_trace[BP_NUM_TABLES]) {
  int r;
  bool given[BP_NUM_TABLES];
  size_t n_given[BP_NUM_TABLES];
  for (int t = 0; t < BP_NUM_TABLES; t++) {
    given[t] = given_table(wit, tcfg, t);
    n_given[t] = given[t] ? wit->n[t] : 0;
  }
  TracePlan plan;
  if ((r = plan_traces(tcfg, given, n_given, &plan))) return r;
  const bool lookup_kf = plan.lookup[L_SPONGE_KECCAK], lookup_bm = plan.lookup[L_PACKING_MEMORY], lookup_sl = plan.lookup[L_SPONGE_LOGIC];
  static const int GEN_ORDER[BP_NUM_TABLES] = {T_KECCAK_SPONGE, T_ARITHMETIC, T_BYTE_PACKING, T_CPU, T_KECCAK, T_LOGIC, T_MEMORY};
  for (int t = 0; t < BP_NUM_TABLES; t++) {
    const uint64_t N = (uint64_t)1 << tcfg[t].log_n;
    d_trace[t] = w.arena.alloc_words((size_t)tcfg[t].n_cols * N);
    if (!d_trace[t]) return fail(BP_ERR_DEVICE, "device arena exhausted (%zu MiB) for table %s", w.arena.capacity() >> 20, TABLES[t].name);
  }
  const uint64_t* d_sponge = d_trace[T_KECCAK_SPONGE];
  const uint32_t sponge_log_n = tcfg[T_KECCAK_SPONGE].log_n;
  const uint64_t sponge_N = (uint64_t)1 << sponge_log_n;
  for (int gi = 0; gi < BP_NUM_TABLES; gi++) {
    const int t = GEN_ORDER[gi];
    const uint64_t N = (uint64_t)1 << tcfg[t].log_n, seed = I[10] ^ splitmix64(t + 1);
    const size_t wds = TABLES[t].item_words, cap = witness_capacity(t, N);
    const size_t mark = w.arena.mark();
    uint64_t* d_in = nullptr;
    if (t == T_LOGIC && lookup_sl) {
      const size_t n_ops = n_given[t], covered = (size_t)air::ctl::SPONGE_LOGIC_OPS * plan.logic_covered;
      d_in = w.arena.alloc_words((size_t)N * wds + n_ops * wds);
      if (!d_in) return fail(BP_ERR_DEVICE, "device arena exhausted for the logic table's operations");
      uint64_t* d_given = nullptr;
      if (n_ops) {
        if (n_ops * wds > w.pinned_words) return fail(BP_ERR_UNSUPPORTED, "too many logic operations for the input staging buffer");
        std::memcpy(w.pinned, wit->in[t], n_ops * wds * 8);
        d_given = d_in + (size_t)N * wds;
        BPG_HIP(hipMemcpyAsync(d_given, w.pinned, n_ops * wds * 8, hipMemcpyHostToDevice, w.stream));
      }
      if ((r = launch_logic_inputs_from_sponge(d_sponge, sponge_log_n, plan.logic_covered, given[t] ? d_given : nullptr, (uint32_t)n_ops,
                                               d_in, (uint32_t)N, seed, w.stream))) return r;
      if (given[t] && !d_given) {
        BPG_HIP(hipMemsetAsync(d_in + covered * wds, 0, ((size_t)N - covered) * wds * 8, w.stream));
      }
    } else if (given[t]) {
      const size_t words = cap * wds;
      d_in = w.arena.alloc_words(words);
      if (!d_in) return fail(BP_ERR_DEVICE, "device arena exhausted for the witness data of table %s", TABLES[t].name);
      if (words > w.pinned_words) return fail(BP_ERR_UNSUPPORTED, "table %s too tall for the input staging buffer", TABLES[t].name);
      fill_table_inputs(t, N, wit->in[t], wit->n[t], w.pinned);
      BPG_HIP(hipMemcpyAsync(d_in, w.pinned, words * 8, hipMemcpyHostToDevice, w.stream));
    } else if (t == T_KECCAK && lookup_kf) {
      d_in = w.arena.alloc_words(cap * wds);
      if (!d_in) return fail(BP_ERR_DEVICE, "device arena exhausted for the Keccak-f table's inputs");
      if ((r = launch_keccak_inputs_from_sponge(d_sponge, sponge_log_n, d_in, (uint32_t)cap, seed, w.stream))) return r;
    } else if (t == T_MEMORY && lookup_bm) {
      d_in = w.arena.alloc_words((size_t)N * wds);
      if (!d_in) return fail(BP_ERR_DEVICE, "device arena exhausted for the memory table's log");
      if ((r = launch_memory_inputs_from_byte_packing(d_trace[T_BYTE_PACKING], tcfg[T_BYTE_PACKING].log_n, d_in, (uint32_t)N, w.stream))) return r;
    }
    r = tcfg[t].air_id == air::SYNTHETIC
            ? launch_synth_trace(d_trace[t], nullptr, tcfg[t].log_n, tcfg[t].n_cols, 0, 1, seed, w.stream)
            : launch_air_trace(tcfg[t].air_id, d_trace[t], d_in, tcfg[t].log_n, d_in ? 0 : seed, w.stream, plan.sponge_row_limit);
    if (r) return r;
    if (t == T_KECCAK && lookup_kf) {
      r = launch_lookup_filter(air::KECCAK_F, d_trace[t], tcfg[t].log_n, d_sponge + (size_t)air::keccak_sponge::COL_FULL * sponge_N,
                               d_sponge + (size_t)air::keccak_sponge::COL_FINAL * sponge_N, (uint32_t)sponge_N, w.stream);
    } else if (t == T_MEMORY && lookup_bm) {
      r = launch_lookup_filter(air::MEMORY, d_trace[t], tcfg[t].log_n, d_trace[T_BYTE_PACKING], nullptr, (uint32_t)1 << tcfg[T_BYTE_PACKING].log_n, w.stream);
    } else if (t == T_LOGIC && lookup_sl) {
      r = launch_lookup_filter(air::LOGIC, d_trace[t], tcfg[t].log_n, d_sponge + (size_t)air::keccak_sponge::COL_FULL * sponge_N,
                               d_sponge + (size_t)air::keccak_sponge::COL_FINAL * sponge_N, plan.logic_covered, w.stream);
    }
    if (r) return r;
    if (d_in) {
      if ((r = w.wait())) return r;
      w.arena.release(mark);
    }
  }
  return BP_OK;
}

static int prove_tables(const bp_state* s, Worker& w, const uint64_t* I, const TxnWitness* wit, TableProofs* tp) {
  StarkCfg* tcfg = tp->tcfg;
  int r;
  uint64_t* d_trace[BP_NUM_TABLES];
  Committed trace[BP_NUM_TABLES];
// ... 542 lines not shown
```

proof_protocol_decoder_amd/csrc/prover.cpp:

```cpp
#include <cstdio>
#include <cstdlib>
#include "prover.hpp"
#include "tune.hpp"
#include <algorithm>
#include <chrono>
#if defined(__x86_64__)
#include <immintrin.h>
#endif
#include <memory>
#include <thread>

namespace bpg {

static const uint64_t RC_HOST[360] = {
#include "poseidon_rc.inc"
};
static inline uint64_t sbox_host(uint64_t x) {
  uint64_t x2 = gl::mulc(x, x), x4 = gl::mulc(x2, x2), x3 = gl::mulc(x2, x);
  return gl::mulc(x3, x4);
}
static const uint32_t MDS_C[12] = {17, 15, 41, 16, 2, 28, 13, 13, 39, 18, 34, 20};
static inline void mds_finish_host(const uint64_t al[12], const uint64_t ah[12], uint64_t s[12]) {
  for (int r = 0; r < 12; r++) {
    const uint64_t l = al[r] + (ah[r] << 32);
// ... 534 lines not shown
      }
    }
    TRY(launch_quotient_chunks(ca, B, st));
  }
  w.arena.release(mark_tmp);
  Committed quot[MAX_BATCH];
  TRY(commit_batch(w, d_qc, Q, B, log_n, r, h, true, quot));
  for (uint32_t b = 0; b < B; b++) {
    std::memcpy(P[b] + L.quot_cap, quot[b].cap.data(), L.cap_words * 8);
    ch[b].observe(quot[b].cap.data(), L.cap_words);
  }
  if (w.aborted()) return fail(BP_ERR_ABORTED, "aborted after quotient commitment");

  gl::Ext zeta[MAX_BATCH], zeta_next[MAX_BATCH];
  for (uint32_t b = 0; b < B; b++) {
    zeta[b] = ch[b].challenge_ext();
    if (gl::eq(gl::pow(zeta[b], N), gl::ext(1))) return fail(BP_ERR_INVALID_INPUT, "Opening point is in the subgroup.");
    zeta_next[b] = gl::scale(zeta[b], wN);
  }

  ARENA_ALLOC(d_pw, (size_t)B * 6 * N);
  {
    PowerVecArgs pv[MAX_BATCH];
    for (uint32_t b = 0; b < B; b++) pv[b] = PowerVecArgs{d_pw + (size_t)b * 6 * N, {zeta[b], zeta_next[b], gl::ext(1)}};
    TRY(launch_power_vectors(pv, B, log_n, 3, st));
  }
  const size_t open_cols = (size_t)K + C + A + Q + A;
  if (open_cols * 4 * B > w.pinned_words) return fail(BP_ERR_UNSUPPORTED, "too many columns for the opening mailbox");
  {
    OpenMulti om[MAX_BATCH] = {};
    for (uint32_t b = 0; b < B; b++) {
      OpenMulti& o = om[b];
      o.stride = N; o.log_n = log_n;
      const uint64_t *pw = d_pw + (size_t)b * 6 * N, *pw1 = pw + 4 * N;
      uint64_t* d_o = w.pinned_dev + (size_t)b * open_cols * 4;
      auto seg = [&](const uint64_t* coeffs, uint32_t n_cols, const uint64_t* pwv, uint32_t n_points) {
        if (n_cols) {
          const uint32_t k = o.n_segs++;
          o.coeffs[k] = coeffs; o.pw[k] = pwv; o.out[k] = d_o; o.n_points[k] = n_points;
          o.first_col[k + 1] = o.first_col[k] + n_cols;
        }
        d_o += (size_t)n_cols * 4;
      };
      seg(K ? consts[b]->coeffs : nullptr, K, pw, 1);
      seg(trace[b].coeffs, C, pw, 2);
      seg(aux[b].coeffs, A, pw, 2);
      seg(quot[b].coeffs, Q, pw, 1);
      seg(aux[b].coeffs, A, pw1, 1);
    }
    TRY(launch_openings_multi(om, B, st));
  }
  TRY(w.wait());
  for (uint32_t b = 0; b < B; b++) {
    const uint64_t* ho = w.pinned + (size_t)b * open_cols * 4;
    uint64_t* oz = P[b] + L.open_zeta;
    for (size_t c = 0; c < (size_t)K + C + A + Q; c++) { oz[2 * c] = ho[4 * c]; oz[2 * c + 1] = ho[4 * c + 1]; }
    uint64_t* on = P[b] + L.open_next;
    for (size_t c = 0; c < (size_t)C + A; c++) { on[2 * c] = ho[4 * (K + c) + 2]; on[2 * c + 1] = ho[4 * (K + c) + 3]; }
    uint64_t* of = P[b] + L.open_first;
    const size_t base = (size_t)K + C + A + Q;
    for (size_t c = 0; c < A; c++) { of[2 * c] = ho[4 * (base + c)]; of[2 * c + 1] = ho[4 * (base + c) + 1]; }
    ch[b].observe(P[b] + L.open_zeta, 2 * (size_t)L.n_zeta);
    ch[b].observe(P[b] + L.open_next, 2 * (size_t)L.n_next);
    ch[b].observe(P[b] + L.open_first, 2 * (size_t)A);
  }

  gl::Ext alpha[MAX_BATCH];
  for (uint32_t b = 0; b < B; b++) alpha[b] = ch[b].challenge_ext();
  const uint32_t k0 = L.n_zeta, k1 = L.n_next, k2 = A;
  ARENA_ALLOC(d_apow, (size_t)B * 2 * k0);
  {
    AlphaPowArgs ap[MAX_BATCH];
    for (uint32_t b = 0; b < B; b++) ap[b] = AlphaPowArgs{d_apow + (size_t)b * 2 * k0, alpha[b]};
    TRY(launch_alpha_pows(ap, B, k0, st));
  }
  struct OracleRef { const Committed* c; int32_t e[3]; };
  OracleRef refs[MAX_BATCH][4];
  int n_or = 0;
  for (uint32_t b = 0; b < B; b++) {
    n_or = 0;
    if (K) refs[b][n_or++] = {consts[b], {0, -1, -1}};
    refs[b][n_or++] = {&trace[b], {(int32_t)K, 0, -1}};
    refs[b][n_or++] = {&aux[b], {(int32_t)(K + C), (int32_t)C, 0}};
    refs[b][n_or++] = {&quot[b], {(int32_t)(K + C + A), -1, -1}};
  }
  const uint32_t cols_per_chunk = 64;
  uint32_t total_chunks = 0;
  for (int o = 0; o < n_or; o++) total_chunks += (refs[0][o].c->n_cols + cols_per_chunk - 1) / cols_per_chunk;
  ARENA_ALLOC(d_g, (size_t)B * 6 * N);
  {
    const bool one_pass = loaded != 0;
    uint64_t* d_cpart = nullptr;
    if (!one_pass) {
      ARENA_ALLOC(cp, (size_t)B * total_chunks * 6 * N);
      d_cpart = cp;
    }
    CombineMulti cm[MAX_BATCH] = {};
    uint64_t* gp[MAX_BATCH];
    CombineReduceArgs cr[MAX_BATCH];
    for (uint32_t b = 0; b < B; b++) {
      uint32_t chunk_base = 0;
      uint64_t* part = d_cpart ? d_cpart + (size_t)b * total_chunks * 6 * N : nullptr;
      for (int o = 0; o < n_or; o++) {
        CombineArgs& cb = cm[b].a[cm[b].n_oracles++];
        cb.coeffs = refs[b][o].c->coeffs; cb.stride = N; cb.log_n = log_n; cb.n_cols = refs[b][o].c->n_cols;
        cb.cols_per_chunk = cols_per_chunk; cb.chunk_base = chunk_base;
        for (int k = 0; k < 3; k++) cb.exp_base[k] = refs[b][o].e[k];
        cb.alpha_pows = d_apow + (size_t)b * 2 * k0; cb.partial = part;
        chunk_base += (cb.n_cols + cols_per_chunk - 1) / cols_per_chunk;
      }
      gp[b] = d_g + (size_t)b * 6 * N;
      cr[b] = CombineReduceArgs{part, gp[b]};
    }
    if (one_pass) {
      TRY(launch_combine_all(cm, B, gp, st));
    } else {
      TRY(launch_combine_partial_multi(cm, B, total_chunks, st));
      TRY(launch_combine_reduce(cr, B, total_chunks, log_n, st));
    }
  }
  ARENA_ALLOC(d_glde, (size_t)B * 6 * M);
  TRY(ntt_br2nat(d_g, N, d_glde, M, N, log_n, 6 * B, R, coset_scale, false, st));
  ARENA_ALLOC(d_v0, (size_t)B * 2 * M);
  {
    FriInitArgs fi[MAX_BATCH] = {};
    for (uint32_t b = 0; b < B; b++) {
      FriInitArgs& f = fi[b];
      f.glde = d_glde + (size_t)b * 6 * M; f.tw_n = tw_n; f.log_n = log_n; f.rate_bits = r;
      std::memcpy(f.g_t, coset.g_t, sizeof(f.g_t));
      const uint64_t* opens[3] = {P[b] + L.open_zeta, P[b] + L.open_next, P[b] + L.open_first};
      const uint32_t kk[3] = {k0, k1, k2};
      for (int k = 0; k < 3; k++) {
        gl::Ext acc = gl::ext(0);
        for (size_t j = kk[k]; j-- > 0;) acc = gl::add(gl::mul(acc, alpha[b]), gl::Ext{opens[k][2 * j], opens[k][2 * j + 1]});
        f.y[k] = acc;
      }
      f.z[0] = zeta[b]; f.z[1] = zeta_next[b]; f.z[2] = gl::ext(1);
      f.alpha_shift[0] = gl::pow(alpha[b], (uint64_t)k1 + k2);
      f.alpha_shift[1] = gl::pow(alpha[b], k2);
      f.alpha_shift[2] = gl::ext(1);
      f.out = d_v0 + (size_t)b * 2 * M;
    }
    TRY(launch_fri_init(fi, B, st));
  }

  const uint32_t ab = cfg.arity_bits, arity = 1u << ab;
  const uint64_t *layer_values[9], *layer_digests[9];
  size_t layer_vstride[9], layer_dstride[9];
  uint32_t layer_log_nl[9];
  uint64_t* cur = d_v0;
  size_t cur_stride = 2 * M;
  uint32_t log_nl = log_n;
  uint64_t shift = gl::GENERATOR;
  for (uint32_t l = 0; l < L.n_layers; l++) {
    const uint32_t log_leaves = log_nl - ab + r;
    const size_t dw = bp_merkle_digest_words(log_leaves, h), next_words = (size_t)2 << log_leaves;
    ARENA_ALLOC(d_dig, dw * B);
    ARENA_ALLOC(d_next, next_words * B);
    FriLayerArgs fa[MAX_BATCH] = {};
    TRY(fri_layer_args(log_nl, r, ab, shift, &fa[0]));
    for (uint32_t b = 0; b < B; b++) {
      if (b) fa[b] = fa[0];
      fa[b].values = cur + b * cur_stride; fa[b].out = d_next + b * next_words; fa[b].digests = d_dig + b * dw;
    }
    TRY(launch_fri_layer_leaves(fa, B, st));
    bool mirrored = false;
    TRY(merkle_upper_levels(d_dig, log_leaves, h, st, w.pinned_dev, &mirrored, B, dw));
    if (!mirrored)
      for (uint32_t b = 0; b < B; b++)
        BPG_HIP(hipMemcpyAsync(w.pinned + b * L.cap_words, d_dig + (b + 1) * dw - L.cap_words, L.cap_words * 8,
                               hipMemcpyDeviceToHost, st));
    TRY(w.wait());
    for (uint32_t b = 0; b < B; b++) {
      uint64_t* cap = P[b] + L.fri_caps + l * L.cap_words;
      std::memcpy(cap, w.pinned + b * L.cap_words, L.cap_words * 8);
      ch[b].observe(cap, L.cap_words);
      fa[b].beta = ch[b].challenge_ext();
    }
    TRY(launch_fri_fold(fa, B, st));
    layer_values[l] = cur; layer_vstride[l] = cur_stride; layer_digests[l] = d_dig; layer_dstride[l] = dw;
    layer_log_nl[l] = log_nl;
    cur = d_next;
    cur_stride = next_words;
    log_nl -= ab;
    shift = gl::pow(shift, arity);
  }
  {
    const uint32_t log_ml = log_nl + r;
    const uint64_t ml = (uint64_t)1 << log_ml, nl = (uint64_t)1 << log_nl;
    if (2 * ml * B > w.pinned_words) return fail(BP_ERR_UNSUPPORTED, "final FRI layer does not fit the mailbox");
    for (uint32_t b = 0; b < B; b++)
      BPG_HIP(hipMemcpyAsync(w.pinned + b * 2 * ml, cur + b * cur_stride, 2 * ml * 8, hipMemcpyDeviceToHost, st));
    TRY(w.wait());
    const uint64_t w_inv = gl::inv(gl::root(log_ml)), s_inv = gl::inv(shift), ml_inv = gl::inv(ml);
    std::vector<uint64_t> wp(ml);
    wp[0] = 1;
    for (uint64_t k = 1; k < ml; k++) wp[k] = gl::mulc(wp[k - 1], w_inv);
    for (uint32_t b = 0; b < B; b++) {
      const uint64_t* hv = w.pinned + b * 2 * ml;
      uint64_t sk = ml_inv;
      for (uint64_t k = 0; k < ml; k++) {
        uint64_t c0 = 0, c1 = 0;
        for (uint64_t i = 0; i < ml; i++) {
          const uint64_t pos = (i & (R - 1)) * nl + (i >> r);
          const uint64_t tw = wp[(i * k) & (ml - 1)];
          c0 = gl::addc(c0, gl::mulc(hv[2 * pos], tw));
          c1 = gl::addc(c1, gl::mulc(hv[2 * pos + 1], tw));
        }
        c0 = gl::mulc(c0, sk);
        c1 = gl::mulc(c1, sk);
        sk = gl::mulc(sk, s_inv);
        if (k < L.final_len) {
          P[b][L.final_poly + 2 * k] = c0;
          P[b][L.final_poly + 2 * k + 1] = c1;
        } else if (c0 || c1) {
          return fail(BP_ERR_INVALID_INPUT, "FRI final polynomial has a non-zero tail: the witness violates the AIR");
        }
      }
      ch[b].observe(P[b] + L.final_poly, 2 * (size_t)L.final_len);
    }
  }
  if (w.aborted()) return fail(BP_ERR_ABORTED, "aborted before proof of work");

  {
    PowArgs pa[MAX_BATCH] = {};
    for (uint32_t b = 0; b < B; b++) {
      ch[b].pow_state(pa[b].state, &pa[b].pos);
      pa[b].bits = cfg.pow_bits;
    }
    unsigned long long res[MAX_BATCH];
    for (uint32_t b = 0; b < B; b++) res[b] = 0;
    if (cfg.pow_bits) {
      const uint32_t batch0 = (uint32_t)std::min<uint64_t>(1u << 20, std::max<uint64_t>(1u << 12, (uint64_t)1 << (cfg.pow_bits ? cfg.pow_bits - 1 : 0)));
      uint32_t batch = batch0, n_batches = 0;
      BPG_HIP(hipMemsetAsync(w.d_pow_result, 0xFF, 8 * MAX_BATCH, st));
      for (uint64_t base = 0;;) {
        for (int k = 0; k < 4; k++) {
          if (++n_batches > 8) batch = std::min<uint32_t>(1u << 20, batch * 2);
          for (uint32_t b = 0; b < B; b++) pa[b].base = base;
          TRY(launch_pow(pa, B, batch, w.d_pow_result, st));
          base += batch;
        }
        BPG_HIP(hipMemcpyAsync(w.pinned, w.d_pow_result, 8 * B, hipMemcpyDeviceToHost, st));
        TRY(w.wait());
        bool all = true;
        for (uint32_t b = 0; b < B; b++) {
          res[b] = reinterpret_cast<const unsigned long long*>(w.pinned)[b];
          all = all && res[b] != ~0ULL;
        }
        if (all) break;
        if (w.aborted()) return fail(BP_ERR_ABORTED, "aborted during proof of work");
        if (base > ((uint64_t)1 << 44)) return fail(BP_ERR_DEVICE, "proof of work search exhausted");
      }
    }
    for (uint32_t b = 0; b < B; b++) {
      const uint64_t nonce = res[b];
      P[b][L.pow] = nonce;
      ch[b].observe(nonce);
      const uint64_t resp = ch[b].challenge();
      if (cfg.pow_bits && (resp >> (64 - cfg.pow_bits)) != 0)
        return fail(BP_ERR_DEVICE, "proof-of-work witness failed the host re-check");
    }
  }

  {
    std::unique_ptr<QueryArgs> qa2(new QueryArgs());
    std::unique_ptr<QueryLayerArgs> ql(new QueryLayerArgs());
    const size_t q_words = (size_t)cfg.num_queries * L.query_words;
    const bool q_direct = q_words * B + 4 * B <= w.pinned_words;
    uint64_t* d_q = q_direct ? w.pinned_dev : w.arena.alloc_words(q_words * B + 4 * B);
    if (!d_q) return fail(BP_ERR_DEVICE, "device arena exhausted (%zu MiB) allocating the query buffer", w.arena.capacity() >> 20);
    qa2->query_words = ql->query_words = L.query_words;
    qa2->n_queries = ql->n_queries = cfg.num_queries;
    qa2->log_n = log_n; qa2->rate_bits = r; qa2->cap_height = h;
    ql->rate_bits = r; ql->cap_height = h; ql->arity_bits = ab;
    for (uint32_t b = 0; b < B; b++) {
      for (uint32_t q = 0; q < cfg.num_queries; q++)
        qa2->x_index[b * cfg.num_queries + q] = ql->x_index[b * cfg.num_queries + q] = ch[b].challenge() & (M - 1);
      qa2->proof[b].out = ql->proof[b].out = d_q + b * q_words;
      qa2->proof[b].first_leaf = first_trace_leaf ? d_q + B * q_words + 4 * b : nullptr;
      uint32_t off = 1;
      for (int o = 0; o < n_or; o++) {
        const Committed* c = refs[b][o].c;
        qa2->proof[b].oracle[o] = QueryOracle{c->lde, c->digests, M, c->n_cols, off};
        off += c->n_cols + L.depth0 * 4;
      }
      for (uint32_t l = 0; l < L.n_layers; l++) {
        ql->proof[b].layer[l] = QueryLayer{layer_values[l] + b * layer_vstride[l], layer_digests[l] + b * layer_dstride[l],
                                          layer_log_nl[l], off};
        off += 2 * arity + (layer_log_nl[l] - ab + r - h) * 4;
      }
    }
    qa2->leaf_oracle = K ? 1 : 0;
    TRY(launch_query_initial(*qa2, B, n_or, st));
    TRY(launch_query_layers(*ql, B, L.n_layers, st));
    if (q_direct) {
      TRY(w.wait());
      for (uint32_t b = 0; b < B; b++) std::memcpy(P[b] + L.queries, w.pinned + b * q_words, q_words * 8);
      if (first_trace_leaf) std::memcpy(first_trace_leaf, w.pinned + B * q_words, 4 * B * 8);
    } else {
      for (uint32_t b = 0; b < B; b++) TRY(w.d2h(P[b] + L.queries, d_q + b * q_words, q_words));
      if (first_trace_leaf) TRY(w.d2h(first_trace_leaf, d_q + B * q_words, 4 * B));
    }
  }
  return BP_OK;
}

}
```

proof_protocol_decoder_amd/csrc/stark_api.cpp:

```cpp
#include <algorithm>
#include <cstdlib>
#include <cstring>
#include <mutex>
#include <string>
#include <vector>
#include "prover.hpp"

using namespace bpg;

namespace {
constexpr uint32_t LONE_PI_LEN = 4;
void lone_public_input_list(uint64_t seed, uint64_t out[LONE_PI_LEN]) {
  for (uint64_t j = 0; j < LONE_PI_LEN; j++) {
    uint64_t z = (seed ^ ((0x50 + j) << 32)) + 0x9E3779B97F4A7C15ULL;
    z = (z ^ (z >> 30)) * 0xBF58476D1CE4E5B9ULL;
    z = (z ^ (z >> 27)) * 0x94D049BB133111EBULL;
    out[j] = gl::canon(z ^ (z >> 31));
  }
}
}
namespace {
std::mutex g_park_mu;
std::vector<Worker*> g_parked;

// ... 661 lines not shown
  return BP_OK;
}
int bp_plonk_constants(uint64_t seed, uint32_t log_n, const bp_plonk_layout* layout, uint64_t* d_consts_out, void* stream) try {
  if (!d_consts_out) return fail(BP_ERR_INVALID_INPUT, "bp_plonk_constants: null output");
  if (log_n < 4 || log_n > 26) return fail(BP_ERR_INVALID_INPUT, "bp_plonk_constants: log_n out of range");
  air::plonk::Layout lay;
  int rc = plonk_layout_of(layout, log_n, &lay);
  if (rc) return rc;
  if ((rc = init_ntt_kernels())) return rc;
  return launch_plonk_constants(d_consts_out, log_n, seed, lay, as_stream(stream));
}
BPG_ABI_CATCH("bp_plonk_constants")
int bp_plonk_trace(const uint64_t* d_consts, uint64_t seed, const uint64_t* pi, const bp_plonk_layout* layout, const uint64_t* paths,
                   uint32_t log_n, uint64_t* d_trace_out, void* stream) try {
  if (!d_consts || !pi || !d_trace_out) return fail(BP_ERR_INVALID_INPUT, "bp_plonk_trace: null argument");
  if (log_n < 4 || log_n > 26) return fail(BP_ERR_INVALID_INPUT, "bp_plonk_trace: log_n out of range");
  air::plonk::Layout lay;
  int rc = plonk_layout_of(layout, log_n, &lay);
  if (rc) return rc;
  if (lay.n_paths && !paths) return fail(BP_ERR_INVALID_INPUT, "bp_plonk_trace: the layout walks %u Merkle paths: their witness is missing", lay.n_paths);
  for (uint32_t j = 0; j < lay.pi_len; j++) if (pi[j] >= gl::P) return fail(BP_ERR_INVALID_INPUT, "bp_plonk_trace: non-canonical public input");
  std::vector<uint64_t> rows, all((size_t)(air::plonk::HASH_ROWS_MAX + air::plonk::merkle_rows(lay) + air::plonk::leaf_rows(lay)) * air::plonk::H_WIRES, 0);
  uint64_t pub[4];
  poseidon_hash_rows(pi, lay.pi_len, &rows, pub);
  std::memcpy(all.data(), rows.data(), rows.size() * 8);
  const uint32_t n_list_rows = (uint32_t)(rows.size() / air::plonk::H_WIRES);
  const size_t path_words = 1 + 4 * (size_t)lay.depth + lay.leaf_len;
  for (uint32_t p = 0; p < lay.n_paths; p++) {
    const uint64_t* pw = paths + p * path_words;
    for (size_t j = 1; j < path_words; j++) if (pw[j] >= gl::P) return fail(BP_ERR_INVALID_INPUT, "bp_plonk_trace: non-canonical sibling word");
    uint64_t root[4];
    poseidon_merkle_rows(pi + lay.path_pi0 + 8 * p, pw[0], pw + 1, lay.depth,
                         all.data() + (size_t)(air::plonk::HASH_ROWS_MAX + p * lay.depth) * air::plonk::H_WIRES, root);
    if (lay.leaf_len) {
      uint64_t digest[4];
      poseidon_hash_rows(pw + 1 + 4 * (size_t)lay.depth, lay.leaf_len, &rows, digest);
      std::memcpy(all.data() + (size_t)(air::plonk::HASH_ROWS_MAX + air::plonk::merkle_rows(lay) + p * air::plonk::hash_rows(lay.leaf_len)) * air::plonk::H_WIRES,
                  rows.data(), rows.size() * 8);
    }
  }
  uint64_t* d_rows = nullptr;
  BPG_HIP(hipMalloc(reinterpret_cast<void**>(&d_rows), all.size() * 8));
  struct Free { uint64_t* p; ~Free() { (void)hipFree(p); } } guard{d_rows};
  BPG_HIP(hipMemcpy(d_rows, all.data(), all.size() * 8, hipMemcpyHostToDevice));
  PlonkTraceArgs a{d_trace_out, d_consts, seed, {pub[0], pub[1], pub[2], pub[3]}, d_rows, n_list_rows,
                   air::plonk::merkle_rows(lay) + air::plonk::leaf_rows(lay), air::plonk::arith_row0(lay)};
  rc = launch_plonk_trace(&a, 1, log_n, as_stream(stream));
  if (rc) return rc;
  BPG_HIP(hipStreamSynchronize(as_stream(stream)));
  return BP_OK;
}
BPG_ABI_CATCH("bp_plonk_trace")


static int quot_cfg(uint32_t air_id, const bp_stark_cfg* shape, StarkCfg* c) {
  if (!shape) return fail(BP_ERR_INVALID_INPUT, "null shape");
  *c = StarkCfg{shape->log_n, shape->n_cols, shape->n_const, shape->deg_pow, shape->rate_bits, shape->cap_height,
                shape->num_queries, shape->pow_bits, shape->arity_bits, shape->final_poly_bits, air_id};
  return check_cfg(*c);
}

uint64_t bp_quotient_scratch_words(uint32_t air_id, const bp_stark_cfg* shape) {
  StarkCfg c;
  if (quot_cfg(air_id, shape, &c)) return 0;
  QuotArgs qa{};
  Ctl ctl{};
  if (init_ntt_kernels()) return 0;
  uint64_t words = 0;
  for (int loaded = 0; loaded < 2; loaded++) {
    if (quotient_args(c, ctl, 1, 1, &qa, nullptr, loaded)) return 0;
    words = std::max<uint64_t>(words, quotient_table_words(qa) + quotient_partial_words(qa));
  }
  return words;
}

int bp_quotient_eval(uint32_t air_id, const bp_stark_cfg* shape, const uint64_t* d_trace_lde, const uint64_t* d_aux_lde,
                     const uint64_t* d_const_lde, const uint64_t ctl_in[4], const uint64_t alphas[2],
                     uint64_t* d_scratch, uint64_t* d_qvals_out, void* stream) try {
  StarkCfg c;
  int rc = quot_cfg(air_id, shape, &c);
  if (rc) return rc;
  if (!d_trace_lde || !d_aux_lde || (c.n_const && !d_const_lde) || !ctl_in || !alphas || !d_scratch || !d_qvals_out)
    return fail(BP_ERR_INVALID_INPUT, "bp_quotient_eval: null argument");
  for (int i = 0; i < 4; i++)
    if (ctl_in[i] >= gl::P) return fail(BP_ERR_INVALID_INPUT, "bp_quotient_eval: non-canonical challenge");
  if (alphas[0] >= gl::P || alphas[1] >= gl::P) return fail(BP_ERR_INVALID_INPUT, "bp_quotient_eval: non-canonical alpha");
  if ((rc = init_ntt_kernels())) return rc;
  Ctl ctl;
  for (int i = 0; i < 4; i++) ctl.v[i] = ctl_in[i];
  QuotArgs qa{};
  QuotCoset coset{};
  qa.trace_lde = d_trace_lde; qa.aux_lde = d_aux_lde; qa.const_lde = c.n_const ? d_const_lde : nullptr;
  if ((rc = quotient_args(c, ctl, alphas[0], alphas[1], &qa, &coset))) return rc;
  qa.apow = d_scratch; qa.partial = d_scratch + quotient_table_words(qa); qa.qvals = d_qvals_out;
  return launch_quotient(qa, coset, as_stream(stream));
}
BPG_ABI_CATCH("bp_quotient_eval")

int bp_air_port_products(uint32_t air_id, const bp_stark_cfg* shape, const uint64_t* d_trace, uint64_t stride, const uint64_t* d_consts,
                         const uint64_t pub[4], const uint64_t ctl_in[4], uint64_t* d_aux_out, void* stream) try {
  const auto program = air::prog::find(air_id);
  if (!program || !program->n_ports)
    return fail(BP_ERR_INVALID_INPUT, "bp_air_port_products: air_id 0x%08x is no registered program with lookup ports", air_id);
  StarkCfg c;
  int rc = quot_cfg(air_id, shape, &c);
  if (rc) return rc;
  if (!d_trace || !ctl_in || !d_aux_out || (c.n_const && !d_consts)) return fail(BP_ERR_INVALID_INPUT, "bp_air_port_products: null argument");
  if (stride < ((uint64_t)1 << c.log_n))
    return fail(BP_ERR_INVALID_INPUT, "bp_air_port_products: column stride %llu is shorter than the 2^%u-row trace", (unsigned long long)stride, c.log_n);
  AuxArgs a{d_trace, d_aux_out, Ctl{}};
  a.consts = c.n_const ? d_consts : nullptr;
  for (int i = 0; i < 4; i++) {
    if (ctl_in[i] >= gl::P || (pub && pub[i] >= gl::P)) return fail(BP_ERR_INVALID_INPUT, "bp_air_port_products: non-canonical challenge or public input");
    a.ctl.v[i] = ctl_in[i];
    a.ctl.pub[i] = pub ? pub[i] : 0;
  }
  if (program->n_public && !pub) return fail(BP_ERR_INVALID_INPUT, "bp_air_port_products: the AIR reads public inputs: pass four words");
  return launch_port_products(&a, 1, air_id, c.log_n, stride, as_stream(stream));
}
BPG_ABI_CATCH("bp_air_port_products")

int bp_debug_air_aux(uint32_t air_id, const bp_stark_cfg* shape, const uint64_t* d_trace, const uint64_t ctl_in[4], uint64_t* d_aux_out,
                     void* stream) try {
  const air::Desc* ai = air::info(air_id);
  if (!ai || !ai->in_pair) return fail(BP_ERR_INVALID_INPUT, "bp_debug_air_aux: air_id %u is no built-in AIR with a lookup side", air_id);
  StarkCfg c;
  int rc = quot_cfg(air_id, shape, &c);
  if (rc) return rc;
  if (!d_trace || !ctl_in || !d_aux_out) return fail(BP_ERR_INVALID_INPUT, "bp_debug_air_aux: null argument");
  AuxArgs a{d_trace, d_aux_out, Ctl{}};
  for (int i = 0; i < 4; i++) {
    if (ctl_in[i] >= gl::P) return fail(BP_ERR_INVALID_INPUT, "bp_debug_air_aux: non-canonical challenge");
    a.ctl.v[i] = ctl_in[i];
  }
  return launch_aux(&a, 1, air_id, c.n_cols, c.log_n, as_stream(stream));
}
BPG_ABI_CATCH("bp_debug_air_aux")

int bp_fri_fold(const uint64_t* d_values, uint32_t log_nl, uint32_t rate_bits, uint32_t arity_bits, uint64_t shift,
                const uint64_t beta[2], uint64_t* d_out, void* stream) try {
  if (!d_values || !d_out || !beta) return fail(BP_ERR_INVALID_INPUT, "bp_fri_fold: null argument");
  if (shift == 0 || shift >= gl::P || beta[0] >= gl::P || beta[1] >= gl::P)
    return fail(BP_ERR_INVALID_INPUT, "bp_fri_fold: non-canonical field element");
  int rc = init_ntt_kernels();
  if (rc) return rc;
  FriLayerArgs fa{};
  if ((rc = fri_layer_args(log_nl, rate_bits, arity_bits, shift, &fa))) return rc;
  fa.values = d_values; fa.out = d_out; fa.digests = nullptr;
  fa.beta = gl::Ext{beta[0], beta[1]};
  return launch_fri_fold(fa, as_stream(stream));
}
BPG_ABI_CATCH("bp_fri_fold")

int bp_pow_grind(const uint64_t state[12], uint32_t pos, uint32_t bits, uint64_t* nonce_out, void* stream) try {
  if (!state || !nonce_out) return fail(BP_ERR_INVALID_INPUT, "bp_pow_grind: null argument");
  if (pos >= 8 || bits == 0 || bits > 40) return fail(BP_ERR_INVALID_INPUT, "bp_pow_grind: pos must be a rate word, bits in 1..40");
  hipStream_t st = as_stream(stream);
  unsigned long long* d_res = nullptr;
  BPG_HIP(hipMalloc(reinterpret_cast<void**>(&d_res), 8));
  PowArgs pa{};
  for (int i = 0; i < 12; i++) pa.state[i] = state[i];
  pa.pos = pos; pa.bits = bits;
  int rc = BP_OK;
  unsigned long long res = ~0ULL;
  if (hipMemsetAsync(d_res, 0xFF, 8, st) != hipSuccess) rc = fail(BP_ERR_DEVICE, "hipMemsetAsync failed");
  uint32_t batch = (uint32_t)std::min<uint64_t>(1u << 20, std::max<uint64_t>(1u << 12, (uint64_t)2 << bits));
  for (uint64_t base = 0; rc == BP_OK; base += batch, batch = std::min<uint32_t>(1u << 20, batch * 2)) {
    pa.base = base;
    if ((rc = launch_pow(pa, batch, d_res, st))) break;
    if (hipMemcpyAsync(&res, d_res, 8, hipMemcpyDeviceToHost, st) != hipSuccess || hipStreamSynchronize(st) != hipSuccess) {
      rc = fail(BP_ERR_DEVICE, "bp_pow_grind: copy back failed");
      break;
    }
    if (res != ~0ULL) break;
    if (base > ((uint64_t)1 << 44)) rc = fail(BP_ERR_DEVICE, "proof of work search exhausted");
  }
  (void)hipFree(d_res);
  if (rc == BP_OK) *nonce_out = res;
  return rc;
}
BPG_ABI_CATCH("bp_pow_grind")

int bp_openings(const uint64_t* d_coeffs, uint64_t stride, uint32_t log_n, uint32_t n_cols, const uint64_t z0[2],
                const uint64_t z1[2], uint64_t* d_pw_scratch, uint64_t* d_out, void* stream) try {
  if (!n_cols) return BP_OK;
  if (!d_coeffs || !z0 || !d_pw_scratch || !d_out) return fail(BP_ERR_INVALID_INPUT, "bp_openings: null argument");
  if (log_n > 30 || stride < ((uint64_t)1 << log_n)) return fail(BP_ERR_INVALID_INPUT, "bp_openings: bad shape");
  const uint64_t* zz[2] = {z0, z1 ? z1 : z0};
  for (int k = 0; k < 2; k++)
    if (zz[k][0] >= gl::P || zz[k][1] >= gl::P) return fail(BP_ERR_INVALID_INPUT, "bp_openings: non-canonical point");
  hipStream_t st = as_stream(stream);
  const uint32_t n_points = z1 ? 2 : 1;
  int rc = launch_power_vectors(d_pw_scratch, log_n, gl::Ext{z0[0], z0[1]}, gl::Ext{zz[1][0], zz[1][1]}, n_points, st);
  if (rc) return rc;
  return launch_openings(d_coeffs, stride, log_n, n_cols, d_pw_scratch, n_points, d_out, st);
}
BPG_ABI_CATCH("bp_openings")

}
```

proof_protocol_decoder_amd/csrc/stark_kernels.hip:

```cpp
#include "common.hpp"
#include "gl.hpp"
#include "poseidon.cuh"
#include "poseidon_mx.cuh"
#include "stark_kernels.hpp"
#include "quotient_dev.cuh"
#include "air_program.hpp"

namespace {

using gl::Ext;
using namespace bpg::k5;

__device__ __forceinline__ uint64_t splitmix64(uint64_t x) {
  uint64_t z = x + 0x9E3779B97F4A7C15ULL;
  z = (z ^ (z >> 30)) * 0xBF58476D1CE4E5B9ULL;
  z = (z ^ (z >> 27)) * 0x94D049BB133111EBULL;
  return z ^ (z >> 31);
}
__device__ __forceinline__ uint64_t rnd(uint64_t seed, uint64_t col, uint64_t row) {
  return gl::canon(splitmix64(seed ^ (col << 32) ^ row));
}
__device__ __forceinline__ uint64_t pow_e(uint64_t t, uint32_t e) {
  return e == 3 ? gl::mulc(gl::mulc(t, t), t) : t;
}
// ... 918 lines not shown
  const bpg::FriLayerArgs& a = batch.a[blockIdx.z];
  const uint32_t log_q = a.log_nl - a.arity_bits;
  const uint64_t n_leaves = (uint64_t)1 << (log_q + a.rate_bits);
  const uint64_t id = blockIdx.x * (uint64_t)blockDim.x + threadIdx.x;
  if (id >= n_leaves) return;
  const uint32_t t = (uint32_t)(id >> log_q), m0 = (uint32_t)(id & ((1u << log_q) - 1));
  const uint64_t base = ((uint64_t)t << a.log_nl) + m0;
  const uint32_t arity = 1u << a.arity_bits;
  uint64_t s[12];
#pragma unroll
  for (int k = 0; k < 12; k++) s[k] = 0;
  for (uint32_t j = 0; j < arity; j += 4) {
#pragma unroll
    for (int u = 0; u < 4; u++) {
      const uint32_t jj = gl::bitrev(j + u, a.arity_bits);
      const uint64_t p = base + ((uint64_t)jj << log_q);
      s[2 * u] = a.values[2 * p];
      s[2 * u + 1] = a.values[2 * p + 1];
    }
    poseidon::permute(s);
  }
  const uint64_t leaf = gl::bitrev((uint32_t)(t + ((uint64_t)m0 << a.rate_bits)), log_q + a.rate_bits);
#pragma unroll
  for (int k = 0; k < 4; k++) a.digests[leaf * 4 + k] = gl::canon(s[k]);
}
__global__ void __launch_bounds__(256) fri_layer_leaf_quad_kernel(bpg::BatchOf<bpg::FriLayerArgs> batch) {
  if (gridDim.x * gridDim.y * gridDim.z <= 64) __builtin_amdgcn_s_setprio(3);
  const bpg::FriLayerArgs& a = batch.a[blockIdx.z];
  __shared__ uint64_t rc[360];
  for (uint32_t i = threadIdx.x; i < 360; i += blockDim.x) rc[i] = poseidon::RC[i];
  __syncthreads();
  const uint32_t log_q = a.log_nl - a.arity_bits;
  const uint64_t n_leaves = (uint64_t)1 << (log_q + a.rate_bits);
  const uint64_t id = (blockIdx.x * (uint64_t)blockDim.x + threadIdx.x) >> 2;
  if (id >= n_leaves) return;
  const poseidon::QuadCtx qc = poseidon::quad_ctx();
  const uint32_t t = (uint32_t)(id >> log_q), m0 = (uint32_t)(id & ((1u << log_q) - 1));
  const uint64_t base = ((uint64_t)t << a.log_nl) + m0;
  const uint32_t arity = 1u << a.arity_bits, u = qc.q >> 1, comp = qc.q & 1;
  uint64_t e[3] = {0, 0, 0};
  for (uint32_t j = 0; j < arity; j += 4) {
    const uint64_t p0 = base + ((uint64_t)gl::bitrev(j + u, a.arity_bits) << log_q);
    const uint64_t p1 = base + ((uint64_t)gl::bitrev(j + 2 + u, a.arity_bits) << log_q);
    e[0] = a.values[2 * p0 + comp];
    e[1] = a.values[2 * p1 + comp];
    poseidon::permute_quad(e, qc, rc);
  }
  const uint64_t leaf = gl::bitrev((uint32_t)(t + ((uint64_t)m0 << a.rate_bits)), log_q + a.rate_bits);
  a.digests[leaf * 4 + qc.q] = gl::canon(e[0]);
}
template <int NS>
__global__ void __launch_bounds__(256) fri_layer_leaf_mx_kernel(bpg::BatchOf<bpg::FriLayerArgs> batch) {
  if (gridDim.x * gridDim.z <= 64) __builtin_amdgcn_s_setprio(3);
  const bpg::FriLayerArgs& a = batch.a[blockIdx.z];
  __shared__ __attribute__((aligned(16))) uint32_t cin[poseidon::mx::CIN_WORDS];
  poseidon::mx::build_cin(cin);
  __syncthreads();
  const poseidon::mx::Ctx c = poseidon::mx::make_ctx(cin);
  const uint32_t log_q = a.log_nl - a.arity_bits;
  const uint64_t n_leaves = (uint64_t)1 << (log_q + a.rate_bits);
  const uint64_t id0 = ((uint64_t)blockIdx.x * 4 + (threadIdx.x >> 6)) * (16 * NS) + (threadIdx.x & 15);
  const uint32_t arity = 1u << a.arity_bits, u = c.kb >> 1, comp = c.kb & 1;
  uint64_t base[NS], e[NS][3];
#pragma unroll
  for (int m = 0; m < NS; m++) {
    const uint64_t id = id0 + 16 * m < n_leaves ? id0 + 16 * m : n_leaves - 1;
    const uint32_t t = (uint32_t)(id >> log_q), m0 = (uint32_t)(id & ((1u << log_q) - 1));
    base[m] = ((uint64_t)t << a.log_nl) + m0;
    e[m][0] = e[m][1] = e[m][2] = 0;
  }
  for (uint32_t j = 0; j < arity; j += 4) {
    const uint64_t o0 = (uint64_t)gl::bitrev(j + u, a.arity_bits) << log_q;
    const uint64_t o1 = (uint64_t)gl::bitrev(j + 2 + u, a.arity_bits) << log_q;
#pragma unroll
    for (int m = 0; m < NS; m++) {
      e[m][0] = a.values[2 * (base[m] + o0) + comp];
      e[m][1] = a.values[2 * (base[m] + o1) + comp];
    }
    poseidon::mx::permute<NS>(e, c);
  }
#pragma unroll
  for (int m = 0; m < NS; m++) {
    const uint64_t id = id0 + 16 * m;
    if (id < n_leaves) {
      const uint32_t t = (uint32_t)(id >> log_q), m0 = (uint32_t)(id & ((1u << log_q) - 1));
      const uint64_t leaf = gl::bitrev((uint32_t)(t + ((uint64_t)m0 << a.rate_bits)), log_q + a.rate_bits);
      a.digests[leaf * 4 + c.kb] = gl::canon(e[m][0]);
    }
  }
}
__global__ void __launch_bounds__(256) fri_fold_kernel(bpg::BatchOf<bpg::FriLayerArgs> batch) {
  if (gridDim.x * gridDim.y * gridDim.z <= 64) __builtin_amdgcn_s_setprio(3);
  const bpg::FriLayerArgs& a = batch.a[blockIdx.z];
  const uint32_t log_q = a.log_nl - a.arity_bits;
  const uint64_t n_out = (uint64_t)1 << (log_q + a.rate_bits);
  const uint64_t id = blockIdx.x * (uint64_t)blockDim.x + threadIdx.x;
  if (id >= n_out) return;
  const uint32_t t = (uint32_t)(id >> log_q), m0 = (uint32_t)(id & ((1u << log_q) - 1));
  const uint64_t base = ((uint64_t)t << a.log_nl) + m0;
  const uint64_t x_inv = gl::mulc(a.g_t_inv[t], root_pow(a.tw_nl_inv, a.log_nl, m0));
  uint64_t c0[16], c1[16];
#pragma unroll
  for (int j = 0; j < 16; j++) {
    const uint64_t p = base + ((uint64_t)j << log_q);
    c0[j] = a.values[2 * p];
    c1[j] = a.values[2 * p + 1];
  }
#pragma unroll
  for (int s = 0; s < 4; s++) {
    const int half = 8 >> s;
#pragma unroll
    for (int k0 = 0; k0 < 8; k0 += 2) {
      uint64_t d[4], w[4], r[4];
      int mm[2];
#pragma unroll
      for (int i = 0; i < 2; i++) {
        const int k = k0 + i, m = (k / half) * 2 * half + (k % half);
        mm[i] = m;
        const uint64_t wv = a.wa_inv_pow[(m & (half - 1)) << s];
        const uint64_t x0 = c0[m], x1 = c1[m], y0 = c0[m + half], y1 = c1[m + half];
        c0[m] = gl::addc(x0, y0);
        c1[m] = gl::addc(x1, y1);
        d[2 * i] = gl::subc(x0, y0);
        d[2 * i + 1] = gl::subc(x1, y1);
        w[2 * i] = wv;
        w[2 * i + 1] = wv;
      }
      if (half == 1) {
#pragma unroll
        for (int i = 0; i < 4; i++) r[i] = d[i];
      } else {
        gl::mul_n<4>(d, w, r);
#pragma unroll
        for (int i = 0; i < 4; i++) r[i] = gl::canon(r[i]);
        __builtin_amdgcn_sched_barrier(0);
      }
#pragma unroll
      for (int i = 0; i < 2; i++) {
        c0[mm[i] + half] = r[2 * i];
        c1[mm[i] + half] = r[2 * i + 1];
      }
    }
  }
  const Ext bx = gl::scale(a.beta, x_inv);
  Ext acc = gl::ext(0);
#pragma unroll
  for (int i = 15; i >= 0; i--) {
    const int slot = ((i & 1) << 3) | ((i & 2) << 1) | ((i & 4) >> 1) | ((i & 8) >> 3);
    acc = gl::add(gl::mul(acc, bx), Ext{c0[slot], c1[slot]});
  }
  acc = gl::scale(acc, a.arity_inv);
  a.out[2 * id] = acc.c0;
  a.out[2 * id + 1] = acc.c1;
}

__global__ void __launch_bounds__(256) pow_grind_kernel(bpg::BatchOf<bpg::PowArgs> batch, unsigned long long* result) {
  const bpg::PowArgs& a = batch.a[blockIdx.z];
  result += blockIdx.z;
  if (__hip_atomic_load(result, __ATOMIC_RELAXED, __HIP_MEMORY_SCOPE_AGENT) < a.base + blockIdx.x * (uint64_t)blockDim.x) return;
  const uint64_t cand = a.base + blockIdx.x * (uint64_t)blockDim.x + threadIdx.x;
  uint64_t s[12];
#pragma unroll
  for (int k = 0; k < 12; k++) s[k] = a.state[k];
  s[a.pos] = cand;
  poseidon::permute(s);
  if ((gl::canon(s[7]) >> (64 - a.bits)) == 0) atomicMin(result, (unsigned long long)cand);
}
template <bool GR>
__global__ void __launch_bounds__(256) __attribute__((amdgpu_waves_per_eu(3)))
pow_grind_mx_kernel(bpg::BatchOf<bpg::PowArgs> batch, unsigned long long* result, const uint32_t* __restrict__ gtab) {
  const bpg::PowArgs& a = batch.a[blockIdx.z];
  result += blockIdx.z;
  __shared__ uint32_t beaten;
  if (threadIdx.x == 0)
    beaten = __hip_atomic_load(result, __ATOMIC_RELAXED, __HIP_MEMORY_SCOPE_AGENT) < a.base + (uint64_t)blockIdx.x * 256;
  __syncthreads();
  if (beaten) return;
  __shared__ __attribute__((aligned(16))) uint32_t cin[GR ? poseidon::mx::CIN_GROUPED_WORDS : poseidon::mx::CIN_WORDS];
  __shared__ __attribute__((aligned(16))) uint32_t gt[GR ? poseidon::mx::grp::TABLE_WORDS : 4];
  if constexpr (GR) {
    poseidon::mx::build_cin_grouped(cin);
    poseidon::mx::grp::load_tables(gt, gtab);
  } else {
    poseidon::mx::build_cin(cin);
  }
  __syncthreads();
  const poseidon::mx::Ctx c = poseidon::mx::make_ctx(cin);
  const uint64_t cand0 = a.base + ((uint64_t)blockIdx.x * 4 + (threadIdx.x >> 6)) * 64 + (threadIdx.x & 15);
  uint64_t e[4][3];
#pragma unroll
  for (int s = 0; s < 3; s++) {
    uint64_t w = a.state[4 * s];
#pragma unroll
    for (int q = 1; q < 4; q++) w = c.kb == (uint32_t)q ? a.state[4 * s + q] : w;
    const bool mine = c.kb + 4 * s == a.pos;
#pragma unroll
    for (int m = 0; m < 4; m++) e[m][s] = mine ? cand0 + 16 * m : w;
  }
  if constexpr (GR) poseidon::mx::permute_grouped(e, c, gt, gtab);
  else poseidon::mx::permute<4>(e, c);
  if (c.kb == 3) {
#pragma unroll
    for (int m = 0; m < 4; m++)
      if ((gl::canon(e[m][1]) >> (64 - a.bits)) == 0) atomicMin(result, (unsigned long long)(cand0 + 16 * m));
  }
}

__global__ void __launch_bounds__(256) query_initial_kernel(bpg::QueryArgs a) {
  if (gridDim.x * gridDim.y * gridDim.z <= 64) __builtin_amdgcn_s_setprio(3);
  const uint32_t b = blockIdx.x / a.n_queries, q = blockIdx.x % a.n_queries, o = blockIdx.y;
  const uint64_t x = a.x_index[blockIdx.x];
  const bpg::QueryOracle& orc = a.proof[b].oracle[o];
  const uint32_t log_rows = a.log_n + a.rate_bits;
  const uint32_t i = gl::bitrev((uint32_t)x, log_rows);
  const uint64_t pos = ((uint64_t)(i & ((1u << a.rate_bits) - 1)) << a.log_n) + (i >> a.rate_bits);
  uint64_t* out = a.proof[b].out;
  if (o == 0 && threadIdx.x == 0) out[(uint64_t)q * a.query_words] = x;
  uint64_t* w = out + (uint64_t)q * a.query_words + orc.out_offset;
  for (uint32_t c = threadIdx.x; c < orc.n_cols; c += blockDim.x) w[c] = orc.lde[(uint64_t)c * orc.stride + pos];
  w += orc.n_cols;
  const uint32_t depth = log_rows - a.cap_height;
  for (uint32_t k = threadIdx.x; k < depth * 4; k += blockDim.x) {
    const uint32_t lvl = k >> 2;
    const uint64_t off = ((uint64_t)2 << log_rows) - ((uint64_t)2 << (log_rows - lvl));
    w[k] = orc.digests[(off + ((x >> lvl) ^ 1)) * 4 + (k & 3)];
  }
  if (q == 0 && o == a.leaf_oracle && a.proof[b].first_leaf && threadIdx.x < 4) a.proof[b].first_leaf[threadIdx.x] = orc.digests[x * 4 + threadIdx.x];
}
__global__ void __launch_bounds__(64) query_layers_kernel(bpg::QueryLayerArgs a) {
  if (gridDim.x * gridDim.y * gridDim.z <= 64) __builtin_amdgcn_s_setprio(3);
  const uint32_t b = blockIdx.x / a.n_queries, q = blockIdx.x % a.n_queries, l = blockIdx.y;
  const bpg::QueryLayer& L = a.proof[b].layer[l];
  const uint32_t arity = 1u << a.arity_bits;
  const uint64_t leaf = a.x_index[blockIdx.x] >> (a.arity_bits * (l + 1));
  const uint32_t log_q = L.log_nl - a.arity_bits, log_leaves = log_q + a.rate_bits;
  const uint32_t c = gl::bitrev((uint32_t)leaf, log_leaves);
  const uint32_t t = c & ((1u << a.rate_bits) - 1), m0 = c >> a.rate_bits;
  const uint64_t base = ((uint64_t)t << L.log_nl) + m0;
  uint64_t* w = a.proof[b].out + (uint64_t)q * a.query_words + L.out_offset;
  for (uint32_t k = threadIdx.x; k < 2 * arity; k += blockDim.x) {
    const uint32_t jj = gl::bitrev(k >> 1, a.arity_bits);
    w[k] = L.values[2 * (base + ((uint64_t)jj << log_q)) + (k & 1)];
  }
  w += 2 * arity;
  const uint32_t depth = log_leaves - a.cap_height;
  for (uint32_t k = threadIdx.x; k < depth * 4; k += blockDim.x) {
    const uint32_t lvl = k >> 2;
    const uint64_t off = ((uint64_t)2 << log_leaves) - ((uint64_t)2 << (log_leaves - lvl));
    w[k] = L.digests[(off + ((leaf >> lvl) ^ 1)) * 4 + (k & 3)];
  }
}

}

namespace bpg {

int launch_synth_constants(uint64_t* d_out, uint32_t log_n, uint32_t n_const, uint64_t seed, hipStream_t st) {
  uint64_t total = (uint64_t)n_const << log_n;
  if (!total) return BP_OK;
  synth_const_kernel<<<ceil_div(total, 256), 256, 0, st>>>(d_out, log_n, n_const, seed);
  BPG_LAUNCH_CHECK();
  return BP_OK;
}
static int check_batch(uint32_t batch) {
  return batch >= 1 && batch <= MAX_BATCH ? BP_OK : fail(BP_ERR_INVALID_INPUT, "batch of %u proofs: 1..%u can be proved in lock-step", batch, MAX_BATCH);
}
int launch_synth_trace(const SynthTraceArgs* a, uint32_t batch, uint32_t log_n, uint32_t n_cols, uint32_t n_const,
                       uint32_t deg_pow, hipStream_t st) {
  if (int rc = check_batch(batch)) return rc;
  dim3 grid(ceil_div((uint64_t)1 << log_n, 256), n_cols / 4 + 1, batch);
  synth_trace_kernel<<<grid, 256, 0, st>>>(batch_of(a, batch), log_n, n_cols, n_const, deg_pow);
  BPG_LAUNCH_CHECK();
  return BP_OK;
}
int launch_air_trace(uint32_t air_id, uint64_t* d_trace, const uint64_t* d_inputs, uint32_t log_n, uint64_t seed, hipStream_t st,
                     uint32_t sponge_row_limit) {
  const unsigned gx = ceil_div((uint64_t)1 << log_n, 256);
  switch (air_id) {
    case air::KECCAK_F: keccak_trace_kernel<<<dim3(gx, 6), 256, 0, st>>>(d_trace, d_inputs, log_n, seed); break;
    case air::LOGIC: logic_trace_kernel<<<dim3(gx, 2), 256, 0, st>>>(d_trace, d_inputs, log_n, seed); break;
    case air::MEMORY: memory_trace_kernel<<<gx, 256, 0, st>>>(d_trace, d_inputs, log_n, seed); break;
    case air::ARITHMETIC: arithmetic_trace_kernel<<<gx, 256, 0, st>>>(d_trace, d_inputs, log_n, seed); break;
    case air::BYTE_PACKING: byte_packing_trace_kernel<<<gx, 256, 0, st>>>(d_trace, d_inputs, log_n, seed); break;
    case air::KECCAK_SPONGE: keccak_sponge_trace_kernel<<<dim3(gx, 3), 256, 0, st>>>(d_trace, d_inputs, log_n, seed, sponge_row_limit); break;
    case air::ARITHMETIC_MUL: arithmetic_mul_trace_kernel<<<gx, 256, 0, st>>>(d_trace, d_inputs, log_n, seed); break;
    default: return fail(BP_ERR_INVALID_INPUT, "launch_air_trace: AIR %u has a witness entry of its own (launch_synth_trace, launch_plonk_trace) or none", air_id);
  }
  BPG_LAUNCH_CHECK();
  return BP_OK;
}
int launch_keccak_inputs_from_sponge(const uint64_t* d_sponge_trace, uint32_t sponge_log_n, uint64_t* d_inputs, uint32_t n_perms,
                                     uint64_t seed, hipStream_t st) {
  if (!n_perms) return BP_OK;
  keccak_inputs_from_sponge_kernel<<<ceil_div(n_perms, 256), 256, 0, st>>>(d_sponge_trace, sponge_log_n, d_inputs, n_perms, seed);
  BPG_LAUNCH_CHECK();
  return BP_OK;
}
int launch_logic_inputs_from_sponge(const uint64_t* d_sponge_trace, uint32_t sponge_log_n, uint32_t covered, const uint64_t* d_given,
                                    uint32_t n_given, uint64_t* d_inputs, uint32_t n_logic, uint64_t seed, hipStream_t st) {
  if (5ull * covered > n_logic || covered > (1u << sponge_log_n))
    return fail(BP_ERR_INVALID_INPUT, "the logic table (%u rows) cannot hold five operations for each of %u sponge rows", n_logic, covered);
  logic_inputs_from_sponge_kernel<<<ceil_div(n_logic, 256), 256, 0, st>>>(d_sponge_trace, sponge_log_n, covered, d_given, n_given, d_inputs,
                                                                           n_logic, seed);
  BPG_LAUNCH_CHECK();
  return BP_OK;
}
// ... 268 lines not shown
```

proof_protocol_decoder_amd/csrc/stark_kernels.hpp:

```cpp
#pragma once
#include <hip/hip_runtime.h>
#include <cstdint>
#include "air.hpp"
#include "gl.hpp"

namespace bpg {

struct Ctl {
  uint64_t v[4];
  uint64_t pub[4] = {0, 0, 0, 0};
};

constexpr uint32_t MAX_BATCH = 8;
template <class A>
struct BatchOf {
  A a[MAX_BATCH];
};
template <class A>
inline BatchOf<A> batch_of(const A* a, uint32_t n) {
  BatchOf<A> b{};
  for (uint32_t i = 0; i < n && i < MAX_BATCH; i++) b.a[i] = a[i];
  return b;
}

struct QuotArgs {
  const uint64_t *trace_lde, *aux_lde, *const_lde;
  uint64_t trace_stride, aux_stride, const_stride;
  uint64_t *partial, *qvals;
  const uint64_t* tw_n;
  const uint64_t* apow;
  uint32_t air_id, log_n, rate_bits, n_cols, n_const, n_aux, deg_pow;
  uint32_t n_air_constraints, n_constraints, n_air_units, n_ctl_units, aux_per_unit, units_per_wg;
  uint32_t side_rows;
  uint32_t n_ports;
  uint64_t alpha0, alpha1, g, g_inv, n_inv;
  Ctl ctl;
};
inline size_t quotient_table_words(const QuotArgs& q) { return 2 * (size_t)q.n_constraints + 48 + (q.n_ports ? 256 : 0); }
struct QuotCoset {
  uint64_t g_t[16], zh_t[16], zh_inv_t[16];
};
struct SynthTraceArgs {
  uint64_t* trace;
  const uint64_t* consts;
  uint64_t seed;
};
struct AuxArgs {
  const uint64_t* trace;
  uint64_t* aux;
  Ctl ctl;
  const uint64_t* consts = nullptr;
};
struct PowerVecArgs {
  uint64_t* out;
  gl::Ext z[3];
};
struct AlphaPowArgs {
  uint64_t* out;
  gl::Ext alpha;
};
struct CombineReduceArgs {
  const uint64_t* partial;
  uint64_t* g;
};
struct ChunkArgs {
  const uint64_t* e;
  const uint64_t* inv_scale;
  uint64_t* out;
  uint64_t out_stride;
  uint32_t log_n, rate_bits;
  uint64_t wr_inv_pow[16];
  uint64_t chunk_scale[16];
};
struct CombineArgs {
  const uint64_t* coeffs;
  uint64_t stride;
  uint32_t log_n, n_cols, cols_per_chunk, chunk_base;
  int32_t exp_base[3];
  const uint64_t* alpha_pows;
  uint64_t* partial;
};
struct CombineMulti {
  CombineArgs a[4];
  uint32_t n_oracles;
};
struct OpenMulti {
  const uint64_t* coeffs[5];
  const uint64_t* pw[5];
  uint64_t* out[5];
  uint32_t first_col[6], n_points[5];
  uint64_t stride;
  uint32_t log_n, n_segs;
};
struct FriInitArgs {
  const uint64_t* glde;
  uint64_t* out;
  const uint64_t* tw_n;
  uint32_t log_n, rate_bits;
  uint64_t g_t[16];
  gl::Ext y[3], z[3], alpha_shift[3];
};
struct FriLayerArgs {
  const uint64_t* values;
  uint64_t* out;
  uint64_t* digests;
  const uint64_t* tw_nl_inv;
  uint32_t log_nl, rate_bits, arity_bits;
  uint64_t g_t_inv[16];
  uint64_t wa_inv_pow[16];
  uint64_t arity_inv;
  gl::Ext beta;
};
struct PowArgs {
  uint64_t state[12];
  uint64_t base;
  uint32_t pos, bits;
};
struct QueryOracle {
  const uint64_t *lde, *digests;
  uint64_t stride;
  uint32_t n_cols, out_offset;
};
constexpr uint32_t MAX_BATCH_QUERIES = 256;
struct QueryProof {
  uint64_t* out;
  QueryOracle oracle[4];
  uint64_t* first_leaf = nullptr;
};
struct QueryArgs {
  uint64_t x_index[MAX_BATCH_QUERIES];
  uint64_t query_words;
  uint32_t log_n, rate_bits, cap_height, n_queries;
  uint32_t leaf_oracle = 0;
  QueryProof proof[MAX_BATCH];
};
struct QueryLayer {
  const uint64_t *values, *digests;
  uint32_t log_nl, out_offset;
};
constexpr uint32_t MAX_FRI_LAYERS = 8;
struct QueryLayerProof {
  uint64_t* out;
  QueryLayer layer[MAX_FRI_LAYERS];
};
struct QueryLayerArgs {
  uint64_t x_index[MAX_BATCH_QUERIES];
  uint64_t query_words;
  uint32_t rate_bits, cap_height, arity_bits, n_queries;
  QueryLayerProof proof[MAX_BATCH];
};

int launch_synth_constants(uint64_t* d_out, uint32_t log_n, uint32_t n_const, uint64_t seed, hipStream_t st);
int launch_synth_trace(const SynthTraceArgs* a, uint32_t batch, uint32_t log_n, uint32_t n_cols, uint32_t n_const,
                       uint32_t deg_pow, hipStream_t st);
inline int launch_synth_trace(uint64_t* d_trace, const uint64_t* d_consts, uint32_t log_n, uint32_t n_cols,
                              uint32_t n_const, uint32_t deg_pow, uint64_t seed, hipStream_t st) {
  const SynthTraceArgs a{d_trace, d_consts, seed};
  return launch_synth_trace(&a, 1, log_n, n_cols, n_const, deg_pow, st);
}
int launch_air_trace(uint32_t air_id, uint64_t* d_trace, const uint64_t* d_inputs, uint32_t log_n, uint64_t seed, hipStream_t st,
                     uint32_t sponge_row_limit = ~0u);
int launch_keccak_inputs_from_sponge(const uint64_t* d_sponge_trace, uint32_t sponge_log_n, uint64_t* d_inputs, uint32_t n_perms,
                                     uint64_t seed, hipStream_t st);
int launch_logic_inputs_from_sponge(const uint64_t* d_sponge_trace, uint32_t sponge_log_n, uint32_t covered, const uint64_t* d_given,
                                    uint32_t n_given, uint64_t* d_inputs, uint32_t n_logic, uint64_t seed, hipStream_t st);
int launch_memory_inputs_from_byte_packing(const uint64_t* d_pack_trace, uint32_t pack_log_n, uint64_t* d_log, uint32_t n_mem,
                                           hipStream_t st);
int launch_lookup_filter(uint32_t air_id, uint64_t* d_trace, uint32_t log_n, const uint64_t* flag_a, const uint64_t* flag_b,
                         uint32_t n_flags, hipStream_t st);
int launch_aux(const AuxArgs* a, uint32_t batch, uint32_t air_id, uint32_t n_cols, uint32_t log_n, hipStream_t st);
int launch_plonk_constants(uint64_t* d_out, uint32_t log_n, uint64_t seed, const air::plonk::Layout& lay, hipStream_t st);
struct PlonkTraceArgs {
  uint64_t* trace;
  const uint64_t* consts;
  uint64_t seed, pub[4];
  const uint64_t* hash_rows;
  uint32_t n_hash_rows;
  uint32_t n_merkle_rows = 0, arith_row0 = (air::plonk::MERKLE_ROW0 + 3) & ~3u;
};
int launch_plonk_trace(const PlonkTraceArgs* a, uint32_t batch, uint32_t log_n, hipStream_t st);
int launch_quotient(const QuotArgs* q, uint32_t batch, const QuotCoset& coset, hipStream_t st);
inline int launch_quotient(const QuotArgs& q, const QuotCoset& coset, hipStream_t st) { return launch_quotient(&q, 1, coset, st); }
struct KernelTimer;
int launch_quotient_program(const BatchOf<QuotArgs>& qb, dim3 grid, KernelTimer& kt, hipStream_t st);
int launch_beta_tables(const BatchOf<QuotArgs>& qb, uint32_t batch, hipStream_t st);
int launch_port_terms(const AuxArgs& a, uint32_t air_id, uint32_t log_n, uint64_t trace_stride, hipStream_t st);
int launch_port_products(const AuxArgs* a, uint32_t batch, uint32_t air_id, uint32_t log_n, uint64_t trace_stride, hipStream_t st);
int launch_quotient_chunks(const ChunkArgs* c, uint32_t batch, hipStream_t st);
int launch_power_vectors(const PowerVecArgs* a, uint32_t batch, uint32_t log_n, uint32_t n_points, hipStream_t st);
inline int launch_power_vectors(uint64_t* d_out, uint32_t log_n, gl::Ext z0, gl::Ext z1, uint32_t n_points,
                                hipStream_t st, gl::Ext z2 = gl::Ext{1, 0}) {
  const PowerVecArgs a{d_out, {z0, z1, z2}};
  return launch_power_vectors(&a, 1, log_n, n_points, st);
}
int launch_alpha_pows(const AlphaPowArgs* a, uint32_t batch, uint32_t count, hipStream_t st);
int launch_openings(const uint64_t* d_coeffs, uint64_t stride, uint32_t log_n, uint32_t n_cols,
                    const uint64_t* d_pw, uint32_t n_points, uint64_t* d_out, hipStream_t st);
int launch_openings_multi(const OpenMulti* m, uint32_t batch, hipStream_t st);
int launch_combine_partial_multi(const CombineMulti* m, uint32_t batch, uint32_t total_chunks, hipStream_t st);
int launch_combine_all(const CombineMulti* m, uint32_t batch, uint64_t* const* d_g, hipStream_t st);
int launch_combine_reduce(const CombineReduceArgs* a, uint32_t batch, uint32_t n_chunks, uint32_t log_n, hipStream_t st);
int launch_fri_init(const FriInitArgs* a, uint32_t batch, hipStream_t st);
int launch_fri_layer_leaves(const FriLayerArgs* a, uint32_t batch, hipStream_t st);
int launch_fri_fold(const FriLayerArgs* a, uint32_t batch, hipStream_t st);
inline int launch_fri_fold(const FriLayerArgs& a, hipStream_t st) { return launch_fri_fold(&a, 1, st); }
int launch_pow(const PowArgs* a, uint32_t batch, uint32_t n_candidates, unsigned long long* d_result, hipStream_t st);
inline int launch_pow(const PowArgs& a, uint32_t n_candidates, unsigned long long* d_result, hipStream_t st) {
  return launch_pow(&a, 1, n_candidates, d_result, st);
}
int launch_query_initial(const QueryArgs& a, uint32_t batch, uint32_t n_oracles, hipStream_t st);
int launch_query_layers(const QueryLayerArgs& a, uint32_t batch, uint32_t n_layers, hipStream_t st);

int init_ntt_kernels();
int get_table(int kind, uint32_t log_n, uint32_t rate_bits, const uint64_t** out);
int intt_nat2br(const uint64_t* in, uint64_t in_stride, uint64_t* out, uint64_t out_stride, uint32_t log_n,
                uint32_t n_cols, bool inverse, hipStream_t st);
int ntt_br2nat(const uint64_t* in, uint64_t in_stride, uint64_t* out, uint64_t out_stride, uint64_t coset_stride,
               uint32_t log_n, uint32_t n_cols, uint32_t n_cosets, const uint64_t* scale, bool inverse,
               hipStream_t st);
const uint32_t* group_tables();
int merkle_upper_levels(uint64_t* d_digests, uint32_t log_leaves, uint32_t cap_height, hipStream_t st,
                        uint64_t* mirror, bool* mirrored, uint32_t batch = 1, uint64_t dig_bstride = 0);
int merkle_commit_cols(const uint64_t* d_lde, uint64_t lde_stride, uint32_t n_cols, uint32_t log_n, uint32_t rate_bits,
                       uint32_t cap_height, uint64_t* d_digests, hipStream_t st, uint64_t* mirror, bool* mirrored,
                       uint32_t batch = 1, uint64_t lde_bstride = 0, uint64_t dig_bstride = 0);

}
```

proof_protocol_decoder_amd/csrc/tune.cpp:

```cpp
#include "tune.hpp"
#include <cstdio>
#include "common.hpp"
#include "stark_kernels.hpp"

namespace bpg {
Tune& tune() {
  static Tune t;
  return t;
}
static_assert(MAX_BATCH == 8, "Tune::rec_batch's default is MAX_BATCH");
}

#define BPG_KNOBS(X)                                                                                            \
  X(quad_threshold) X(assume_loaded) X(merkle_fused) X(merkle_wide) X(poseidon_mx) X(poseidon_mx_sets)          \
  X(poseidon_grouped) X(ntt_mx) X(ntt_split) X(k5_spread) X(host_wait) X(host_poseidon) X(rec_batch)            \
  X(witness_threads) X(side_lanes)

extern "C" {

void bp_tune_quad_threshold(uint64_t n_perms) { bpg::tune().quad_threshold.store(n_perms); }
void bp_tune_assume_loaded(int mode) { bpg::tune().assume_loaded.store(mode < 0 ? -1 : (mode != 0)); }
void bp_tune_merkle_fused(int mode) { bpg::tune().merkle_fused.store(mode < 0 ? -1 : (mode != 0)); }
void bp_tune_merkle_wide(int log2_parents) { bpg::tune().merkle_wide.store(log2_parents < 8 || log2_parents > 24 ? 0 : log2_parents); }
void bp_tune_poseidon_mx(int on) { bpg::tune().poseidon_mx.store(on != 0); }
void bp_tune_poseidon_mx_sets(int sets) { bpg::tune().poseidon_mx_sets.store(sets == 1 || sets == 2 || sets == 4 ? sets : 0); }
void bp_tune_poseidon_grouped(int on) { bpg::tune().poseidon_grouped.store(on != 0); }
void bp_tune_ntt_mx(int mode) { bpg::tune().ntt_mx.store(mode < 0 || mode > 3 ? 3 : mode); }
void bp_tune_ntt_split(int mode) { bpg::tune().ntt_split.store(mode == 1 || mode == 2 ? mode : 0); }
void bp_tune_k5_spread(int on) { bpg::tune().k5_spread.store(on != 0); }
void bp_tune_host_wait(int mode) { bpg::tune().host_wait.store(mode < 0 || mode > 2 ? 0 : mode); }
void bp_tune_host_poseidon(int mode) { bpg::tune().host_poseidon.store(mode == 1 ? 1 : 0); }
void bp_tune_rec_batch(int n) { bpg::tune().rec_batch.store(n < 1 ? 1 : (n > (int)bpg::MAX_BATCH ? (int)bpg::MAX_BATCH : n)); }
void bp_tune_witness_threads(int n) { bpg::tune().witness_threads.store(n < 1 ? 1 : (n > 16 ? 16 : n)); }
void bp_tune_side_lanes(int n) { bpg::tune().side_lanes.store(n < 0 ? 0 : n); }
void bp_tune_rec_riders(int on) { bpg::tune().rec_riders.store(on != 0); }

void bp_tune_reset(void) {
  const bpg::Tune defaults;
  bpg::Tune& t = bpg::tune();
#define X(k) t.k.store(defaults.k.load());
  BPG_KNOBS(X)
#undef X
  t.rec_riders.store(defaults.rec_riders.load());
}

int bp_debug_tune_state(char* buf, size_t cap) {
  if (!buf || !cap) return bpg::fail(BP_ERR_INVALID_INPUT, "bp_debug_tune_state: no buffer");
  const bpg::Tune& t = bpg::tune();
  size_t n = 0;
#define X(k)                                                                                   \
  if (n < cap) {                                                                               \
    const int w = std::snprintf(buf + n, cap - n, #k "=%lld\n", (long long)t.k.load());         \
    n += w > 0 ? (size_t)w : 0;                                                                \
  }
  BPG_KNOBS(X)
#undef X
  if (n >= cap) return bpg::fail(BP_ERR_INVALID_INPUT, "bp_debug_tune_state: buffer of %zu bytes is too small", cap);
  return BP_OK;
}

}
```

proof_protocol_decoder_amd/csrc/tune.hpp:

```cpp
#pragma once
#include <atomic>
#include <cstdint>

namespace bpg {

struct Tune {
  std::atomic<uint64_t> quad_threshold{0};
  std::atomic<int> assume_loaded{-1};
  std::atomic<int> merkle_fused{1};
  std::atomic<int> merkle_wide{0};
  std::atomic<int> poseidon_mx{1};
  std::atomic<int> poseidon_mx_sets{0};
  std::atomic<int> poseidon_grouped{1};

  std::atomic<int> ntt_mx{3};
  std::atomic<int> ntt_split{0};

  std::atomic<int> k5_spread{0};
  std::atomic<int> host_wait{0};
  std::atomic<int> host_poseidon{0};
  std::atomic<int> rec_batch{8};
  std::atomic<int> witness_threads{7};
  std::atomic<int> side_lanes{1};

  std::atomic<int> rec_riders{1};
};

Tune& tune();

}
```

Before: 35.21.

## Add planned Merkle tail kernels and mirror final FRI layer to pinned memory

Reworks the Merkle upper-level builder into a step plan, adding a multi-level middle kernel and an LDS-chained cap kernel so the tree tail needs fewer launches when queues are oversubscribed. The new tail path sits behind a merkle_tail knob whose default of 0 leaves the old plan in use. The FRI fold kernel can now also write the last layer straight into pinned host memory, which drops the separate device-to-host copies. That path runs whenever the layer fits in the pinned buffer, in exchange for extra writes from the kernel into host-visible memory.

```diff
diff --git a/include/bpg.h b/include/bpg.h
--- a/include/bpg.h
+++ b/include/bpg.h
@@ -46,6 +46,16 @@
 void bp_tune_quad_threshold(uint64_t n_perms);
 void bp_tune_merkle_fused(int mode);
 void bp_tune_merkle_wide(int log2_parents);
+void bp_tune_merkle_tail(int mode);
+int bp_debug_merkle_plan(uint32_t log_leaves, uint32_t cap_height, uint32_t batch, int loaded, int few_queues,
+                         uint32_t* out, uint32_t max_steps);
+int bp_debug_fri_fold_batch(const uint64_t* d_values, uint64_t values_bstride, uint32_t log_nl, uint32_t rate_bits,
+                            uint32_t arity_bits, uint64_t shift, const uint64_t* betas, uint64_t* d_out, uint64_t out_bstride,
+                            uint64_t* d_mirror, uint32_t batch, void* stream);
+int bp_debug_merkle_commit_batch(const uint64_t* d_lde, uint64_t lde_stride, uint32_t n_cols, uint32_t log_n,
+                                 uint32_t rate_bits, uint32_t cap_height, uint64_t* d_digests, uint32_t batch,
+                                 uint64_t lde_bstride, uint64_t dig_bstride, uint64_t* d_mirror, int* mirrored,
+                                 void* stream);
 void bp_tune_poseidon_mx(int on);
 void bp_tune_poseidon_mx_sets(int sets);
 void bp_tune_poseidon_grouped(int on);
diff --git a/proof_protocol_decoder_amd/_lib.py b/proof_protocol_decoder_amd/_lib.py
--- a/proof_protocol_decoder_amd/_lib.py
+++ b/proof_protocol_decoder_amd/_lib.py
@@ -138,6 +138,11 @@
     L.bp_tune_reset.argtypes = []
     L.bp_tune_reset.restype = None
     L.bp_debug_tune_state.argtypes = [C.c_char_p, C.c_size_t]
+    L.bp_tune_merkle_tail.argtypes = [i]
+    L.bp_tune_merkle_tail.restype = None
+    L.bp_debug_merkle_plan.argtypes = [u32, u32, u32, i, i, C.POINTER(u32), u32]
+    L.bp_debug_fri_fold_batch.argtypes = [vp, u64, u32, u32, u32, u64, C.POINTER(u64), vp, u64, vp, u32, vp]
+    L.bp_debug_merkle_commit_batch.argtypes = [vp, u64, u32, u32, u32, u32, vp, u32, u64, u64, vp, C.POINTER(i), vp]
     _lib = L
     return L
 
diff --git a/proof_protocol_decoder_amd/csrc/hash_kernels.hip b/proof_protocol_decoder_amd/csrc/hash_kernels.hip
--- a/proof_protocol_decoder_amd/csrc/hash_kernels.hip
+++ b/proof_protocol_decoder_amd/csrc/hash_kernels.hip
@@ -434,6 +434,126 @@
   }
 }
 
+template <bool GR>
+__global__ void BPG_MX_BOUNDS
+merkle_middle_kernel(uint64_t* lvl, uint64_t n_parents, uint32_t wg_parents0, uint32_t levels, uint64_t dig_bstride,
+                     const uint32_t* __restrict__ gtab) {
+  if (gridDim.x * gridDim.z <= 64) __builtin_amdgcn_s_setprio(3);
+  lvl += blockIdx.z * dig_bstride;
+  BPG_MX_TABLES(4, GR, gtab)
+  const poseidon::mx::Ctx c = poseidon::mx::make_ctx(cin);
+  const uint32_t wave = threadIdx.x >> 6, n = threadIdx.x & 15;
+  uint64_t level_parents = n_parents;
+  uint32_t wg_parents = wg_parents0;
+  uint64_t wg_first = (uint64_t)blockIdx.x * wg_parents0;
+  const uint64_t* src = lvl;
+  uint64_t* dst = lvl + level_parents * 8;
+  for (uint32_t l = 0; l < levels; l++) {
+    for (uint32_t q0 = wave * 64; q0 < wg_parents; q0 += 256) {
+      uint64_t e[4][3];
+#pragma unroll
+      for (int m = 0; m < 4; m++) {
+        const uint32_t q = q0 + 16 * m + n;
+        const uint64_t i = wg_first + (q < wg_parents ? q : wg_parents - 1);
+        e[m][0] = src[i * 8 + c.kb];
+        e[m][1] = src[i * 8 + 4 + c.kb];
+        e[m][2] = 0;
+      }
+      if constexpr (GR) {
+        uint32_t lane = threadIdx.x & 63;
+        asm volatile("" : "+v"(lane));
+        poseidon::mx::permute_grouped(e, c, gt, gtab, lane);
+      } else {
+        poseidon::mx::permute<4>(e, c);
+      }
+#pragma unroll
+      for (int m = 0; m < 4; m++) {
+        const uint32_t q = q0 + 16 * m + n;
+        if (q < wg_parents) {
+          const uint64_t d = gl::canon(e[m][0]);
+          dst[(wg_first + q) * 4 + c.kb] = d;
+        }
+      }
+    }
+    __syncthreads();
+    src = dst;
+    dst += level_parents * 4;
+    level_parents >>= 1;
+    wg_parents >>= 1;
+    wg_first >>= 1;
+  }
+}
+
+__global__ void __launch_bounds__(256)
+merkle_cap_kernel(const uint64_t* __restrict__ child, uint64_t* __restrict__ out, uint64_t n_parents, uint32_t wg_parents0,
+                  uint32_t levels, uint64_t* __restrict__ mirror, uint64_t dig_bstride) {
+  if (gridDim.x * gridDim.z <= 64) __builtin_amdgcn_s_setprio(3);
+  child += blockIdx.z * dig_bstride;
+  out += blockIdx.z * dig_bstride;
+  if (mirror) mirror += blockIdx.z * ((n_parents >> (levels - 1)) * 4);
+  __shared__ __attribute__((aligned(16))) uint32_t cin[poseidon::mx::CIN_WORDS];
+  __shared__ uint64_t sm[2][128 * 4];
+  poseidon::mx::build_cin(cin);
+  __syncthreads();
+  const poseidon::mx::Ctx c = poseidon::mx::make_ctx(cin);
+  const uint32_t wave = threadIdx.x >> 6, n = threadIdx.x & 15;
+  uint64_t level_parents = n_parents;
+  uint32_t wg_parents = wg_parents0;
+  uint64_t wg_first = (uint64_t)blockIdx.x * wg_parents0;
+  uint64_t* dst = out;
+  for (uint32_t l = 0; l < levels; l++) {
+    const uint64_t* prev = sm[(l - 1) & 1];
+    const bool cap = mirror && l + 1 == levels;
+    if (wg_parents == 128) {
+      uint64_t e[2][3];
+#pragma unroll
+      for (int m = 0; m < 2; m++) {
+        const uint32_t q = wave * 32 + 16 * m + n;
+        if (l == 0) {
+          e[m][0] = child[(wg_first + q) * 8 + c.kb];
+          e[m][1] = child[(wg_first + q) * 8 + 4 + c.kb];
+        } else {
+          e[m][0] = prev[(2 * q) * 4 + c.kb];
+          e[m][1] = prev[(2 * q + 1) * 4 + c.kb];
+        }
+        e[m][2] = 0;
+      }
+      poseidon::mx::permute<2>(e, c);
+#pragma unroll
+      for (int m = 0; m < 2; m++) {
+        const uint32_t q = wave * 32 + 16 * m + n;
+        const uint64_t d = gl::canon(e[m][0]);
+        dst[(wg_first + q) * 4 + c.kb] = d;
+        if (cap) mirror[(wg_first + q) * 4 + c.kb] = d;
+        sm[l & 1][q * 4 + c.kb] = d;
+      }
+    } else if (wave * 16 < wg_parents) {
+      const uint32_t q = wave * 16 + n, qc = q < wg_parents ? q : wg_parents - 1;
+      uint64_t e[1][3];
+      if (l == 0) {
+        e[0][0] = child[(wg_first + qc) * 8 + c.kb];
+        e[0][1] = child[(wg_first + qc) * 8 + 4 + c.kb];
+      } else {
+        e[0][0] = prev[(2 * qc) * 4 + c.kb];
+        e[0][1] = prev[(2 * qc + 1) * 4 + c.kb];
+      }
+      e[0][2] = 0;
+      poseidon::mx::permute<1>(e, c);
+      if (q < wg_parents) {
+        const uint64_t d = gl::canon(e[0][0]);
+        dst[(wg_first + q) * 4 + c.kb] = d;
+        if (cap) mirror[(wg_first + q) * 4 + c.kb] = d;
+        sm[l & 1][q * 4 + c.kb] = d;
+      }
+    }
+    __syncthreads();
+    dst += level_parents * 4;
+    level_parents >>= 1;
+    wg_parents >>= 1;
+    wg_first >>= 1;
+  }
+}
+
 template <int K>
 __device__ __forceinline__ void mul_pow2_planes(const uint64_t (&x)[4], uint64_t* __restrict__ out, uint64_t n, uint64_t i0) {
   uint64_t r4[4], r3[3];
@@ -540,20 +660,21 @@
   return a < 0 ? g_active_provers.load(std::memory_order_relaxed) >= 6 : a != 0;
 }
 bool poseidon_mx() { return tune().poseidon_mx.load(std::memory_order_relaxed) != 0; }
-uint64_t quad_threshold() {
+static uint64_t quad_threshold_at(bool loaded) {
   const uint64_t t = tune().quad_threshold.load(std::memory_order_relaxed);
   if (t) return t;
-  const bool loaded = device_loaded();
   if (poseidon_mx()) return (uint64_t)1 << (loaded ? 13 : 19);
   return (uint64_t)1 << (loaded ? 13 : 17);
 }
-int mx_sets(uint64_t n) {
+uint64_t quad_threshold() { return quad_threshold_at(device_loaded()); }
+static int mx_sets_at(uint64_t n, bool loaded) {
   if (!poseidon_mx()) return 0;
   const int f = tune().poseidon_mx_sets.load(std::memory_order_relaxed);
   if (f) return f;
-  const uint64_t t = quad_threshold();
+  const uint64_t t = quad_threshold_at(loaded);
   return n >= t ? 4 : (n >= t / 2 ? 2 : 1);
 }
+int mx_sets(uint64_t n) { return mx_sets_at(n, device_loaded()); }
 static std::mutex g_group_mu;
 static const uint32_t* g_group_dev[16] = {};
 static std::atomic<int> g_group_state[16];
@@ -634,60 +755,105 @@
     default: KERNEL<1, false><<<dim3(ceil_div((ITEMS), 64), 1, (BATCH)), 256, 0, st>>>(__VA_ARGS__, nullptr); break; \
   }
 
+static std::atomic<int> g_few_queues{0};
+void set_few_queues(bool few) { g_few_queues.store(few, std::memory_order_relaxed); }
+bool few_queues() { return g_few_queues.load(std::memory_order_relaxed) != 0; }
+
+int merkle_plan(uint32_t log_leaves, uint32_t cap_height, uint32_t batch, bool loaded, bool few, MerkleStep* out,
+                uint32_t max_steps) {
+  uint32_t n = 0, l = log_leaves;
+  auto push = [&](uint32_t kernel, uint32_t levels, uint32_t wg_parents, uint32_t sets) {
+    if (n < max_steps) out[n] = MerkleStep{kernel, l, levels, wg_parents, sets};
+    n++;
+    l -= levels;
+  };
+  if (l <= cap_height) return 0;
+  const int fmode = tune().merkle_fused.load(std::memory_order_relaxed);
+  const int wide = tune().merkle_wide.load(std::memory_order_relaxed);
+  const int tail = tune().merkle_tail.load(std::memory_order_relaxed);
+  const bool mx = poseidon_mx();
+  const uint64_t qt = quad_threshold_at(loaded);
+
+  if (mx && fmode != 0 && wide == 0 && (tail > 0 || (tail < 0 && few))) {
+    const uint32_t max_launches = log_leaves <= 12 ? 2 : 3;
+    const int forced = tune().poseidon_mx_sets.load(std::memory_order_relaxed);
+    uint32_t r = l - cap_height;
+    const uint64_t stated = tune().quad_threshold.load(std::memory_order_relaxed), fill = stated ? stated : (uint64_t)1 << 17;
+    while (r > 0) {
+      const bool fills = ((uint64_t)1 << (l - 1)) * batch >= fill;
+      const uint32_t after = r - 1, launches = n + 1 + (after == 0 ? 0 : after <= 8 ? 1 : 2);
+      if (!(r > 19 || (fills && launches <= max_launches))) break;
+      const uint32_t ns = forced ? (uint32_t)forced : 4;
+      push(MK_LEVEL_MX, 1, 64 * ns, ns);
+      r--;
+    }
+    if (r > 8) {
+      const uint32_t m = r - 8;
+      push(MK_MIDDLE, m, 256u << (m > 9 ? m - 9 : 0), 4);
+      r = 8;
+    }
+    if (r > 0) {
+      const uint32_t wg = l - 1 >= 7 ? 128u : 1u << (l - 1);
+      push(MK_CAP, r, wg, wg == 128 ? 2 : 1);
+    }
+    return (int)n;
+  }
+
+  while (l > cap_height) {
+    const uint64_t parents = (uint64_t)1 << (l - 1);
+    constexpr uint64_t flimit = 2048;
+    const bool fused = parents <= flimit && parents < qt && (fmode > 0 || (fmode < 0 && !loaded));
+    if (!fused && fmode > 0 && mx && parents >= 256 && parents <= ((uint64_t)1 << wide) && parents % 256 == 0) {
+      push(MK_WIDE, l - cap_height > 9 ? 9 : l - cap_height, 256, 4);
+    } else if (!fused) {
+      if (const int ns = mx_sets_at(parents * batch, loaded)) push(MK_LEVEL_MX, 1, 64 * ns, ns);
+      else if (parents * batch >= qt) push(MK_LEVEL_LANE, 1, 256, 0);
+      else push(MK_LEVEL_QUAD, 1, 64, 0);
+    } else {
+      const uint32_t wg = parents >= 64 ? 64 : (uint32_t)parents;
+      uint32_t levels = l - cap_height, max_levels = 1;
+      for (uint32_t p = wg; p > 1; p >>= 1) max_levels++;
+      if (levels > max_levels) levels = max_levels;
+      push(mx ? MK_SUBTREE_MX : MK_SUBTREE_QUAD, levels, wg, mx ? 1 : 0);
+    }
+  }
+  return (int)n;
+}
+
 int merkle_upper_levels(uint64_t* d_digests, uint32_t log_leaves, uint32_t cap_height, hipStream_t st,
                         uint64_t* mirror, bool* mirrored, uint32_t batch, uint64_t dig_bstride) {
-  uint64_t* lvl = d_digests;
-  uint32_t l = log_leaves;
   if (mirrored) *mirrored = false;
   if (batch == 0 || batch > MAX_BATCH) return fail(BP_ERR_INVALID_INPUT, "merkle: batch of %u trees", batch);
-  while (l > cap_height) {
+  MerkleStep plan[32];
+  const int n_steps = merkle_plan(log_leaves, cap_height, batch, device_loaded(), few_queues(), plan, 32);
+  if (n_steps < 0 || n_steps > 32) return fail(BP_ERR_INVALID_INPUT, "merkle: no plan for 2^%u leaves", log_leaves);
+  uint64_t* lvl = d_digests;
+  for (int k = 0; k < n_steps; k++) {
+    const MerkleStep& s = plan[k];
+    const uint32_t l = s.first;
     const uint64_t cnt = (uint64_t)1 << l, parents = cnt / 2;
     uint64_t* nxt = lvl + cnt * 4;
-    const int fmode = tune().merkle_fused.load(std::memory_order_relaxed);
-    constexpr uint64_t flimit = 2048;
-    const bool fused = parents <= flimit && parents < quad_threshold() && (fmode > 0 || (fmode < 0 && !device_loaded()));
-    const uint64_t wlimit = (uint64_t)1 << tune().merkle_wide.load(std::memory_order_relaxed);
-    if (!fused && fmode > 0 && poseidon_mx() && parents >= 256 && parents <= wlimit && parents % 256 == 0) {
-      uint32_t levels = l - cap_height;
-      if (levels > 9) levels = 9;
-      uint64_t* mir = (l - levels == cap_height) ? mirror : nullptr;
-      merkle_subtree_wide_kernel<<<dim3((uint32_t)(parents / 256), 1, batch), 256, 0, st>>>(lvl, nxt, parents, levels, mir, dig_bstride);
-      BPG_LAUNCH_CHECK();
-      if (mir && mirrored) *mirrored = true;
-      for (uint32_t k = 0; k < levels; k++) {
-        lvl += ((uint64_t)1 << l) * 4;
-        l--;
-      }
-      continue;
-    }
-    if (!fused) {
-      uint64_t* mir = (l - 1 == cap_height) ? mirror : nullptr;
-      if (const int ns = mx_sets(parents * batch)) {
-        BPG_MX_DISPATCH(ns, merkle_level_mx_kernel, parents, batch, lvl, nxt, parents, mir, dig_bstride)
-      } else if (parents * batch >= quad_threshold())
-        merkle_level_kernel<<<dim3(ceil_div(parents, 256), 1, batch), 256, 0, st>>>(lvl, nxt, parents, mir, dig_bstride);
-      else
-        merkle_level_quad_kernel<<<dim3(ceil_div(cnt * 2, 256), 1, batch), 256, 0, st>>>(lvl, nxt, parents, mir, dig_bstride);
-      BPG_LAUNCH_CHECK();
-      if (mir && mirrored) *mirrored = true;
-      lvl = nxt;
-      l--;
-      continue;
-    }
-    uint32_t levels = l - cap_height;
-    const uint32_t wgs = parents >= 64 ? (uint32_t)(parents / 64) : 1;
-    uint32_t max_levels = 1;
-    for (uint64_t p = parents >= 64 ? 64 : parents; p > 1; p >>= 1) max_levels++;
-    if (levels > max_levels) levels = max_levels;
-    uint64_t* mir = (l - levels == cap_height) ? mirror : nullptr;
-    if (poseidon_mx()) merkle_subtree_mx_kernel<<<dim3(wgs, 1, batch), 256, 0, st>>>(lvl, nxt, parents, levels, mir, dig_bstride);
-    else merkle_subtree_quad_kernel<<<dim3(wgs, 1, batch), 256, 0, st>>>(lvl, nxt, parents, levels, mir, dig_bstride);
+    uint64_t* mir = (l - s.levels == cap_height) ? mirror : nullptr;
+    const dim3 wgs((uint32_t)ceil_div(parents, s.wg_parents), 1, batch);
+    switch (s.kernel) {
+      case MK_LEVEL_MX: BPG_MX_DISPATCH((int)s.sets, merkle_level_mx_kernel, parents, batch, lvl, nxt, parents, mir, dig_bstride) break;
+      case MK_LEVEL_LANE: merkle_level_kernel<<<wgs, 256, 0, st>>>(lvl, nxt, parents, mir, dig_bstride); break;
+      case MK_LEVEL_QUAD: merkle_level_quad_kernel<<<wgs, 256, 0, st>>>(lvl, nxt, parents, mir, dig_bstride); break;
+      case MK_SUBTREE_MX: merkle_subtree_mx_kernel<<<wgs, 256, 0, st>>>(lvl, nxt, parents, s.levels, mir, dig_bstride); break;
+      case MK_SUBTREE_QUAD: merkle_subtree_quad_kernel<<<wgs, 256, 0, st>>>(lvl, nxt, parents, s.levels, mir, dig_bstride); break;
+      case MK_WIDE: merkle_subtree_wide_kernel<<<wgs, 256, 0, st>>>(lvl, nxt, parents, s.levels, mir, dig_bstride); break;
+      case MK_MIDDLE:
+        if (const uint32_t* gtab = group_tables())
+          merkle_middle_kernel<true><<<wgs, 256, 0, st>>>(lvl, parents, s.wg_parents, s.levels, dig_bstride, gtab);
+        else
+          merkle_middle_kernel<false><<<wgs, 256, 0, st>>>(lvl, parents, s.wg_parents, s.levels, dig_bstride, nullptr);
+        break;
+      case MK_CAP: merkle_cap_kernel<<<wgs, 256, 0, st>>>(lvl, nxt, parents, s.wg_parents, s.levels, mir, dig_bstride); break;
+      default: return fail(BP_ERR_INVALID_INPUT, "merkle: plan step of kind %u", s.kernel);
+    }
     BPG_LAUNCH_CHECK();
     if (mir && mirrored) *mirrored = true;
-    for (uint32_t k = 0; k < levels; k++) {
-      lvl += ((uint64_t)1 << l) * 4;
-      l--;
-    }
+    for (uint32_t j = 0; j < s.levels; j++) lvl += ((uint64_t)1 << (l - j)) * 4;
   }
   return BP_OK;
 }
@@ -773,6 +939,28 @@
                                  bpg::as_stream(stream), nullptr, nullptr, 1, 0, 0);
 }
 BPG_ABI_CATCH("bp_merkle_commit")
+
+int bp_debug_merkle_commit_batch(const uint64_t* d_lde, uint64_t lde_stride, uint32_t n_cols, uint32_t log_n,
+                                 uint32_t rate_bits, uint32_t cap_height, uint64_t* d_digests, uint32_t batch,
+                                 uint64_t lde_bstride, uint64_t dig_bstride, uint64_t* d_mirror, int* mirrored,
+                                 void* stream) try {
+  bool m = false;
+  const int rc = bpg::merkle_commit_cols(d_lde, lde_stride, n_cols, log_n, rate_bits, cap_height, d_digests,
+                                         bpg::as_stream(stream), d_mirror, &m, batch, lde_bstride, dig_bstride);
+  if (mirrored) *mirrored = m;
+  return rc;
+}
+BPG_ABI_CATCH("bp_debug_merkle_commit_batch")
+
+int bp_debug_merkle_plan(uint32_t log_leaves, uint32_t cap_height, uint32_t batch, int loaded, int few_queues,
+                         uint32_t* out, uint32_t max_steps) {
+  if (log_leaves > 30 || cap_height > log_leaves || batch == 0 || batch > bpg::MAX_BATCH || (max_steps && !out))
+    return bpg::fail(BP_ERR_INVALID_INPUT, "bp_debug_merkle_plan: bad shape (log_leaves=%u cap_height=%u batch=%u)",
+                     log_leaves, cap_height, batch);
+  static_assert(sizeof(bpg::MerkleStep) == 5 * sizeof(uint32_t), "five words per step");
+  return bpg::merkle_plan(log_leaves, cap_height, batch, loaded != 0, few_queues != 0,
+                          reinterpret_cast<bpg::MerkleStep*>(out), max_steps);
+}
 
 }
 
diff --git a/proof_protocol_decoder_amd/csrc/poseidon_mx.cuh b/proof_protocol_decoder_amd/csrc/poseidon_mx.cuh
--- a/proof_protocol_decoder_amd/csrc/poseidon_mx.cuh
+++ b/proof_protocol_decoder_amd/csrc/poseidon_mx.cuh
@@ -354,9 +354,9 @@
     dst[i] = src[i < 4 * CIN_PER_ROUND / 4 ? i : i + (30 - CIN_GROUPED_ROUNDS) * CIN_PER_ROUND / 4];
 }
 
-__device__ __forceinline__ void mds4_lds(uint64_t (&e)[4][3], const Ctx& c, int rnd, const uint32_t* tab) {
+__device__ __forceinline__ void mds4_lds(uint64_t (&e)[4][3], const Ctx& c, int rnd, const uint32_t* tab, uint32_t lane) {
   const v4i* cr = (const v4i*)(c.cin + cin_slot(rnd) * CIN_PER_ROUND);
-  const v4i* am = (const v4i*)(tab + grp::OPS_WORDS + grp::N_GROUPS * grp::C_WORDS) + (threadIdx.x & 63);
+  const v4i* am = (const v4i*)(tab + grp::OPS_WORDS + grp::N_GROUPS * grp::C_WORDS) + lane;
 #pragma unroll
   for (int m = 0; m < 4; m++) {
     v4i blo, bhi;
@@ -381,7 +381,7 @@
 }
 
 __device__ __forceinline__ void permute_grouped(uint64_t (&e)[4][3], const Ctx& c, const uint32_t* tab,
-                                                const uint32_t* __restrict__ gtab) {
+                                                const uint32_t* __restrict__ gtab, uint32_t lane = threadIdx.x & 63) {
 #pragma unroll
   for (int a = 0; a < 3; a++) {
     const uint64_t k = RC[c.kb + 4 * a];
@@ -392,18 +392,18 @@
 #pragma unroll 1
   for (int k = 0; k < 4; k++, rnd++) {
     sbox_full<4>(e);
-    mds4_lds(e, c, rnd, tab);
+    mds4_lds(e, c, rnd, tab, lane);
   }
   grp::State s;
   grp::init_state(s);
-  grp::Lanes o = grp::lanes_of(threadIdx.x & 63);
+  grp::Lanes o = grp::lanes_of(lane);
 #pragma unroll 1
   for (int g = 0; g < grp::N_GROUPS; g++) grp::partial_group(s, o, e, tab, gtab, g);
   rnd = 26;
 #pragma unroll 1
   for (int k = 0; k < 4; k++, rnd++) {
     sbox_full<4>(e);
-    mds4_lds(e, c, rnd, tab);
+    mds4_lds(e, c, rnd, tab, lane);
   }
 }
 
diff --git a/proof_protocol_decoder_amd/csrc/proofgen.cpp b/proof_protocol_decoder_amd/csrc/proofgen.cpp
--- a/proof_protocol_decoder_amd/csrc/proofgen.cpp
+++ b/proof_protocol_decoder_amd/csrc/proofgen.cpp
@@ -486,6 +486,7 @@
   {
     const char* env = std::getenv("GPU_MAX_HW_QUEUES");
     const long queues = env && *env ? std::strtol(env, nullptr, 10) : 4;
+    set_few_queues(queues < (long)cfg->n_workers);
     if (queues < (long)cfg->n_workers) {
       char buf[512];
       std::snprintf(buf, sizeof(buf),
diff --git a/proof_protocol_decoder_amd/csrc/prover.cpp b/proof_protocol_decoder_amd/csrc/prover.cpp
--- a/proof_protocol_decoder_amd/csrc/prover.cpp
+++ b/proof_protocol_decoder_amd/csrc/prover.cpp
@@ -710,6 +710,7 @@
   size_t cur_stride = 2 * M;
   uint32_t log_nl = log_n;
   uint64_t shift = gl::GENERATOR;
+  bool final_mirrored = false;
   for (uint32_t l = 0; l < L.n_layers; l++) {
     const uint32_t log_leaves = log_nl - ab + r;
     const size_t dw = bp_merkle_digest_words(log_leaves, h), next_words = (size_t)2 << log_leaves;
@@ -735,6 +736,10 @@
       ch[b].observe(cap, L.cap_words);
       fa[b].beta = ch[b].challenge_ext();
     }
+    if (l + 1 == L.n_layers && next_words * B <= w.pinned_words) {
+      for (uint32_t b = 0; b < B; b++) fa[b].mirror = w.pinned_dev + b * next_words;
+      final_mirrored = true;
+    }
     TRY(launch_fri_fold(fa, B, st));
     layer_values[l] = cur; layer_vstride[l] = cur_stride; layer_digests[l] = d_dig; layer_dstride[l] = dw;
     layer_log_nl[l] = log_nl;
@@ -747,8 +752,9 @@
     const uint32_t log_ml = log_nl + r;
     const uint64_t ml = (uint64_t)1 << log_ml, nl = (uint64_t)1 << log_nl;
     if (2 * ml * B > w.pinned_words) return fail(BP_ERR_UNSUPPORTED, "final FRI layer does not fit the mailbox");
-    for (uint32_t b = 0; b < B; b++)
-      BPG_HIP(hipMemcpyAsync(w.pinned + b * 2 * ml, cur + b * cur_stride, 2 * ml * 8, hipMemcpyDeviceToHost, st));
+    if (!final_mirrored)
+      for (uint32_t b = 0; b < B; b++)
+        BPG_HIP(hipMemcpyAsync(w.pinned + b * 2 * ml, cur + b * cur_stride, 2 * ml * 8, hipMemcpyDeviceToHost, st));
     TRY(w.wait());
     const uint64_t w_inv = gl::inv(gl::root(log_ml)), s_inv = gl::inv(shift), ml_inv = gl::inv(ml);
     std::vector<uint64_t> wp(ml);
diff --git a/proof_protocol_decoder_amd/csrc/stark_api.cpp b/proof_protocol_decoder_amd/csrc/stark_api.cpp
--- a/proof_protocol_decoder_amd/csrc/stark_api.cpp
+++ b/proof_protocol_decoder_amd/csrc/stark_api.cpp
@@ -837,6 +837,29 @@
 }
 BPG_ABI_CATCH("bp_fri_fold")
 
+int bp_debug_fri_fold_batch(const uint64_t* d_values, uint64_t values_bstride, uint32_t log_nl, uint32_t rate_bits,
+                            uint32_t arity_bits, uint64_t shift, const uint64_t* betas, uint64_t* d_out, uint64_t out_bstride,
+                            uint64_t* d_mirror, uint32_t batch, void* stream) try {
+  if (!d_values || !d_out || !betas) return fail(BP_ERR_INVALID_INPUT, "bp_debug_fri_fold_batch: null argument");
+  if (batch == 0 || batch > MAX_BATCH) return fail(BP_ERR_INVALID_INPUT, "bp_debug_fri_fold_batch: batch of %u", batch);
+  if (shift == 0 || shift >= gl::P) return fail(BP_ERR_INVALID_INPUT, "bp_debug_fri_fold_batch: non-canonical shift");
+  int rc = init_ntt_kernels();
+  if (rc) return rc;
+  FriLayerArgs fa[MAX_BATCH] = {};
+  if ((rc = fri_layer_args(log_nl, rate_bits, arity_bits, shift, &fa[0]))) return rc;
+  const uint64_t out_words = (uint64_t)2 << (log_nl - arity_bits + rate_bits);
+  for (uint32_t b = 0; b < batch; b++) {
+    if (betas[2 * b] >= gl::P || betas[2 * b + 1] >= gl::P)
+      return fail(BP_ERR_INVALID_INPUT, "bp_debug_fri_fold_batch: non-canonical beta");
+    if (b) fa[b] = fa[0];
+    fa[b].values = d_values + b * values_bstride; fa[b].out = d_out + b * out_bstride;
+    fa[b].mirror = d_mirror ? d_mirror + b * out_words : nullptr;
+    fa[b].beta = gl::Ext{betas[2 * b], betas[2 * b + 1]};
+  }
+  return launch_fri_fold(fa, batch, as_stream(stream));
+}
+BPG_ABI_CATCH("bp_debug_fri_fold_batch")
+
 int bp_pow_grind(const uint64_t state[12], uint32_t pos, uint32_t bits, uint64_t* nonce_out, void* stream) try {
   if (!state || !nonce_out) return fail(BP_ERR_INVALID_INPUT, "bp_pow_grind: null argument");
   if (pos >= 8 || bits == 0 || bits > 40) return fail(BP_ERR_INVALID_INPUT, "bp_pow_grind: pos must be a rate word, bits in 1..40");
diff --git a/proof_protocol_decoder_amd/csrc/stark_kernels.hip b/proof_protocol_decoder_amd/csrc/stark_kernels.hip
--- a/proof_protocol_decoder_amd/csrc/stark_kernels.hip
+++ b/proof_protocol_decoder_amd/csrc/stark_kernels.hip
@@ -1094,6 +1094,10 @@
   acc = gl::scale(acc, a.arity_inv);
   a.out[2 * id] = acc.c0;
   a.out[2 * id + 1] = acc.c1;
+  if (a.mirror) {
+    a.mirror[2 * id] = acc.c0;
+    a.mirror[2 * id + 1] = acc.c1;
+  }
 }
 
 __global__ void __launch_bounds__(256) pow_grind_kernel(bpg::BatchOf<bpg::PowArgs> batch, unsigned long long* result) {
diff --git a/proof_protocol_decoder_amd/csrc/stark_kernels.hpp b/proof_protocol_decoder_amd/csrc/stark_kernels.hpp
--- a/proof_protocol_decoder_amd/csrc/stark_kernels.hpp
+++ b/proof_protocol_decoder_amd/csrc/stark_kernels.hpp
@@ -110,6 +110,7 @@
   uint64_t wa_inv_pow[16];
   uint64_t arity_inv;
   gl::Ext beta;
+  uint64_t* mirror = nullptr;
 };
 struct PowArgs {
   uint64_t state[12];
@@ -219,6 +220,19 @@
                uint32_t log_n, uint32_t n_cols, uint32_t n_cosets, const uint64_t* scale, bool inverse,
                hipStream_t st);
 const uint32_t* group_tables();
+enum MerkleKernel : uint32_t {
+  MK_LEVEL_MX = 0, MK_LEVEL_LANE = 1, MK_LEVEL_QUAD = 2,
+  MK_SUBTREE_MX = 3, MK_SUBTREE_QUAD = 4,
+  MK_WIDE = 5,
+  MK_MIDDLE = 6, MK_CAP = 7
+};
+struct MerkleStep {
+  uint32_t kernel, first, levels, wg_parents, sets;
+};
+int merkle_plan(uint32_t log_leaves, uint32_t cap_height, uint32_t batch, bool loaded, bool few, MerkleStep* out,
+                uint32_t max_steps);
+void set_few_queues(bool few);
+bool few_queues();
 int merkle_upper_levels(uint64_t* d_digests, uint32_t log_leaves, uint32_t cap_height, hipStream_t st,
                         uint64_t* mirror, bool* mirrored, uint32_t batch = 1, uint64_t dig_bstride = 0);
 int merkle_commit_cols(const uint64_t* d_lde, uint64_t lde_stride, uint32_t n_cols, uint32_t log_n, uint32_t rate_bits,
diff --git a/proof_protocol_decoder_amd/csrc/tune.cpp b/proof_protocol_decoder_amd/csrc/tune.cpp
--- a/proof_protocol_decoder_amd/csrc/tune.cpp
+++ b/proof_protocol_decoder_amd/csrc/tune.cpp
@@ -34,6 +34,7 @@
 void bp_tune_witness_threads(int n) { bpg::tune().witness_threads.store(n < 1 ? 1 : (n > 16 ? 16 : n)); }
 void bp_tune_side_lanes(int n) { bpg::tune().side_lanes.store(n < 0 ? 0 : n); }
 void bp_tune_rec_riders(int on) { bpg::tune().rec_riders.store(on != 0); }
+void bp_tune_merkle_tail(int mode) { bpg::tune().merkle_tail.store(mode < 0 ? -1 : (mode != 0)); }
 
 void bp_tune_reset(void) {
   const bpg::Tune defaults;
@@ -42,6 +43,7 @@
   BPG_KNOBS(X)
 #undef X
   t.rec_riders.store(defaults.rec_riders.load());
+  t.merkle_tail.store(defaults.merkle_tail.load());
 }
 
 int bp_debug_tune_state(char* buf, size_t cap) {
diff --git a/proof_protocol_decoder_amd/csrc/tune.hpp b/proof_protocol_decoder_amd/csrc/tune.hpp
--- a/proof_protocol_decoder_amd/csrc/tune.hpp
+++ b/proof_protocol_decoder_amd/csrc/tune.hpp
@@ -9,6 +9,7 @@
   std::atomic<int> assume_loaded{-1};
   std::atomic<int> merkle_fused{1};
   std::atomic<int> merkle_wide{0};
+  std::atomic<int> merkle_tail{0};
   std::atomic<int> poseidon_mx{1};
   std::atomic<int> poseidon_mx_sets{0};
   std::atomic<int> poseidon_grouped{1};
```

Result: no change. 35.15 (-0.2%).
